# HliasGit/navier_stokes_solver

Measured on AMD Instinct MI355X. Metric: DoF*iters/s (FGMRES+aSIMPLE, Re=100; first K=5 outer iterations), higher is better.
Workload: dtype f64

## Files before the change

### navier_stokes_solver_amd/csrc/nsk_capi.cpp

```cpp
#include <rccl/rccl.h>

#include <algorithm>
#include <cstring>

#include "../../include/nsk_threads.h"
#include <omp.h>
#include "nsk_handle.hpp"
#include "nsk_internal.h"

extern "C" {

int nsk_get_unique_id(void *out128) {
  ncclUniqueId id;
  if (ncclGetUniqueId(&id) != ncclSuccess) return -20;
  std::memcpy(out128, &id, sizeof(id));
  return 0;
}

int nsk_local_group_id(int nranks, void *out128) {
  if (nranks < 1 || !out128) return -1;
  make_local_group(nranks, out128, 0);
  return 0;
}

// ... 45 lines not shown
  S.n = (int)(e - b);
  S.ng = n_ghost;
  S.gbegin = b;
  S.gend = e;
  S.ghost_gid.assign(gids, gids + n_ghost);
  h->support[space].clear();
  h->tF_ok = h->tMp_ok = h->tS_ok = false;
  return 0;
  NSK_CATCH(h)
}

int nsk_set_support_points(nsk_handle h, int space, const double *xy) {
  NSK_TRY(h)
  if (space < 0 || space > 1) throw Error(-50, "nsk_set_support_points: bad space");
  const Space &S = h->sp[space];
  if (xy) h->support[space].assign(xy, xy + 2 * (size_t)S.n);
  else h->support[space].clear();
  h->tF_ok = h->tMp_ok = h->tS_ok = false;
  return 0;
  NSK_CATCH(h)
}

int nsk_set_halo_plan(nsk_handle h, int space, int nn, const int32_t *peer, const int32_t *send_ptr,
                      const int32_t *send_idx, const int32_t *recv_ptr) {
  NSK_TRY_DEV(h)
  if (space < 0 || space > 1 || nn < 0) throw Error(-52, "nsk_set_halo_plan: bad arguments");
  Space &S = h->sp[space];
  S.peers.assign(peer, peer + nn);
  S.send_ptr.assign(send_ptr, send_ptr + nn + 1);
  S.recv_ptr.assign(recv_ptr, recv_ptr + nn + 1);
  S.n_send = nn ? send_ptr[nn] : 0;
  for (int k = 0; k < S.n_send; ++k)
    if (send_idx[k] < 0 || send_idx[k] >= S.n) throw Error(-53, "halo plan: send index outside the owned range");
  if (nn && recv_ptr[nn] != S.ng) throw Error(-54, "halo plan: receive counts do not cover the ghost list");
  S.d_send_idx.upload(send_idx, (size_t)S.n_send, h->s());
  S.d_send_buf.alloc((size_t)std::max(1, S.n_send));
  h->ctx.sync();
  return 0;
  NSK_CATCH(h)
}

int nsk_set_block_csr(nsk_handle h, int b, int n_rows, int n_cols, const int32_t *rowptr, const int32_t *col,
                      const double *val) {
  NSK_TRY_DEV(h)
  if (b < 0 || b > NSK_BLK_BT_GHOST) throw Error(-55, "nsk_set_block_csr: bad block id");
  const int rs = (b == NSK_BLK_F || b == NSK_BLK_BT) ? 0 : 1;
  const int cs = (b == NSK_BLK_F || b == NSK_BLK_B) ? 0 : 1;
  const Space &R = h->sp[rs], &Cc = h->sp[cs];
  const int want_rows = b == NSK_BLK_BT_GHOST ? h->sp[0].ng : R.n;
  if (n_rows != want_rows) throw Error(-56, "nsk_set_block_csr: row count does not match the partition");
  if (n_cols != Cc.n + Cc.ng) throw Error(-57, "nsk_set_block_csr: column count does not match owned+ghost");
  const int64_t nnz = rowptr[n_rows];
  for (int i = 0; i < n_rows; ++i)
    if (rowptr[i + 1] < rowptr[i]) throw Error(-58, "nsk_set_block_csr: rowptr not monotone");
  bool bad_col = false;
#pragma omp parallel for schedule(static) reduction(|| : bad_col)
  for (int64_t k = 0; k < nnz; ++k) bad_col = bad_col || col[k] < 0 || col[k] >= n_cols;
  if (bad_col) throw Error(-59, "nsk_set_block_csr: column id out of range");
  Csr &A = h->blk[b];
  Phase ph("hand-off of one block");
  A.n_rows = n_rows;
  A.n_cols = n_cols;
  A.n_own_cols = Cc.n;
  A.nnz = nnz;
  A.h_rowptr.assign(rowptr, rowptr + n_rows + 1);
  A.h_col.resize((size_t)nnz);
#pragma omp parallel for schedule(static)
  for (int64_t c = 0; c < (nnz + (1 << 20) - 1) >> 20; ++c)
    std::memcpy(A.h_col.data() + (c << 20), col + (c << 20), sizeof(int) * (size_t)std::min<int64_t>(1 << 20, nnz - (c << 20)));
  A.rowptr.upload(rowptr, (size_t)n_rows + 1, h->s());
  A.col.upload(col, (size_t)nnz, h->s());
  A.val.upload(val, (size_t)nnz, h->s());
  if (b == NSK_BLK_MP) ++h->mp_values_version;
  ++A.values_version;
  A.release_f32();
  if (b == NSK_BLK_F) h->asmd.mf_valid = false;
  A.lpr = pick_lpr(nnz, n_rows);
  A.present = true;
  A.build_stream_plan(h->s());
  if (b == NSK_BLK_MP) h->index16_for(A, "M_p");
  if (b == NSK_BLK_F) A.build_blocked(2, 2, h->s());
  if (b == NSK_BLK_BT) A.build_blocked(2, 1, h->s());
  if (b == NSK_BLK_B) A.build_blocked(1, 2, h->s());
  h->ctx.sync();
  if (b == NSK_BLK_F || b == NSK_BLK_BT) { h->jrow_ok = h->jblk_ok = false; h->jrow_nblk = h->jblk_nblk = 0; }
  if (b == NSK_BLK_F) {
    h->tF_ok = false;
    h->amgF.clear();
    if (h->amg_active) h->amg_pending = true;
  }
  if (b == NSK_BLK_MP) h->tMp_ok = false;
  if (b == NSK_BLK_B || b == NSK_BLK_BT || b == NSK_BLK_BT_GHOST) { h->s_symbolic = false; h->tS_ok = false; }
  return 0;
  NSK_CATCH(h)
}

int nsk_update_values(nsk_handle h, int b, const double *val) {
  NSK_TRY_DEV(h)
  if (b < 0 || b > NSK_BLK_BT_GHOST || !h->blk[b].present) throw Error(-60, "nsk_update_values: block not set");
  Csr &A = h->blk[b];
  NSK_HIP(hipMemcpyAsync(A.val.p, val, sizeof(double) * (size_t)A.nnz, hipMemcpyHostToDevice, h->s()));
  if (b == NSK_BLK_MP) ++h->mp_values_version;
  if (b == NSK_BLK_F) h->asmd.mf_valid = false;
  ++A.values_version;
  A.refresh_blocked(h->s());
  h->ctx.sync();
  return 0;
  NSK_CATCH(h)
}

int nsk_set_option(nsk_handle h, int opt, double v) {
  NSK_TRY(h)
  switch (opt) {
    case NSK_OPT_TRI_ORDERING: h->tri_ordering = v != 0.0 ? ORDER_MULTICOLOR : ORDER_NATURAL; break;
    case NSK_OPT_SUBDOMAINS: h->subdomains = std::max(1, (int)v); break;
    case NSK_OPT_FUSE_BLOCK_ROW: h->fuse_block_row = v != 0.0; break;
    case NSK_OPT_STREAM_KERNELS: h->use_stream = v != 0.0; break;
    case NSK_OPT_TRI_SYNC_FREE:
      if (v != 0.0 && v != 1.0 && v != 2.0) throw Error(-61, "NSK_OPT_TRI_SYNC_FREE: 0, 1 or 2");
      h->sync_free_mode = (int)v;
      break;
    case NSK_IOPT_FAULT_INJECT:
      h->fault_inject = (int)v;
      h->ctx.mgs_fault = (h->fault_inject & 4) != 0;
      break;
    case NSK_OPT_TRI_LINE_GROUPS:
      if (v != 0.0 && v != 1.0 && v != 2.0) throw Error(-61, "NSK_OPT_TRI_LINE_GROUPS: 0, 1 or 2");
      h->line_groups = (int)v;
      break;
    case NSK_OPT_MASS_ORDERING:
      if (v != -1.0 && v != 0.0 && v != 1.0) throw Error(-61, "NSK_OPT_MASS_ORDERING: -1, 0 or 1");
      h->mp_ordering = (int)v;
      break;
    case NSK_IOPT_GROUP_U:
    case NSK_IOPT_GROUP_P:
      if (v < 1.0 || v > (double)kTriGroupMax) throw Error(-61, "line-group size: 1 .. 3");
      (opt == NSK_IOPT_GROUP_U ? h->group_u : h->group_p) = (int)v;
      break;
    case NSK_IOPT_FUSED_MGS: h->ctx.fused_mgs = v != 0.0; break;
    case NSK_IOPT_GS_ONE_LAUNCH:
      if (v != 0.0 && v != 1.0 && v != 2.0) throw Error(-61, "one-launch Gram-Schmidt sweeps: 0, 1 or 2");
      h->ctx.gs_one_launch = (int)v;
      break;
    case NSK_IOPT_FGMRES_SKIP_UNUSED:
      if (v != 0.0 && v != 1.0) throw Error(-61, "NSK_IOPT_FGMRES_SKIP_UNUSED: 0 or 1");
      h->skip_unused = v != 0.0;
      break;
    case NSK_IOPT_OVERLAP_HALO: h->overlap_halo = v != 0.0; break;
    case NSK_IOPT_TINY_BYTES: h->tF.tiny_bytes = h->tMp.tiny_bytes = h->tS.tiny_bytes = v; break;
    case NSK_OPT_BSR_VELOCITY: h->use_bsr = v != 0.0; break;
    case NSK_OPT_VELOCITY_AMG: h->velocity_amg = v != 0.0; break;
    case NSK_IOPT_TIMEOP_BETWEEN: h->timeop_between = (int)v; break;
    case NSK_IOPT_INDEX16:
      h->index16 = v != 0.0;
      (void)hipSetDevice(h->ctx.device);
      for (int b : {NSK_BLK_MP, NSK_BLK_S})
        if (h->blk[b].present && h->blk[b].stream_ok) h->index16_for(h->blk[b], b == NSK_BLK_S ? "S" : "M_p");
      h->ctx.sync();
      h->tS_ok = h->tMp_ok = false;
      break;
    case NSK_IOPT_HOST_ANALYSIS:
      h->tF.host_analysis = h->tS.host_analysis = h->tMp.host_analysis = v != 0.0;
      h->tF_ok = h->tS_ok = h->tMp_ok = false;
      break;
    case NSK_OPT_BLAS1_PAIRS:
      if (v != -1.0 && v != 0.0 && v != 1.0) throw Error(-61, "NSK_OPT_BLAS1_PAIRS: -1, 0 or 1");
      h->blas1_pairs = (int)v;
      h->ctx.ws.pairs = v < 0.0 ? (h->variant == 0) : (int)v;
      break;
    case NSK_OPT_SCHUR_SIGN:
      if (v != 1.0 && v != -1.0) throw Error(-61, "NSK_OPT_SCHUR_SIGN: +1 or -1");
      h->schur_sign = (int)v;
      break;
    case NSK_OPT_FACTOR_PRECISION:
      if (v != 64.0 && v != 32.0) throw Error(-61, "NSK_OPT_FACTOR_PRECISION: 64 or 32");
      h->factor_precision = (int)v;
      break;
    case NSK_OPT_INNER_MATRIX_PRECISION:
      if (v != 64.0 && v != 32.0) throw Error(-61, "NSK_OPT_INNER_MATRIX_PRECISION: 64 or 32");
      h->inner_matrix_precision = (int)v;
      break;
    case NSK_OPT_INNER_BASIS_PRECISION:
      if (v != 64.0 && v != 32.0) throw Error(-61, "NSK_OPT_INNER_BASIS_PRECISION: 64 or 32");
      h->inner_basis_precision = (int)v;
      break;
    case NSK_OPT_AMG_PRECISION:
      if (v != 64.0 && v != 32.0) throw Error(-61, "NSK_OPT_AMG_PRECISION: 64 or 32");
      h->amg_precision = (int)v;
      break;
    case NSK_OPT_INNER_MATRIX_FREE_F:
      if (v != 0.0 && v != 1.0) throw Error(-61, "NSK_OPT_INNER_MATRIX_FREE_F: 0 or 1");
      h->matrix_free_f = (int)v;
      break;
    case NSK_IOPT_TRI_X_LAYOUT:
      h->x_layout_mode = v == 0.0 ? 0 : 2;
      h->tF_ok = false;
      break;
    case NSK_OPT_INNER_FUSED_GS:
      if (v != 0.0 && v != 1.0 && v != 2.0) throw Error(-61, "NSK_OPT_INNER_FUSED_GS: 0, 1 or 2");
      h->inner_fused_gs = (int)v;
      break;
    case NSK_OPT_OUTER_FUSED_GS: h->outer_fused_gs = v != 0.0; break;
    case NSK_OPT_CG_SINGLE_REDUCTION: h->cg_fused = v != 0.0; break;
    default: throw Error(-61, "nsk_set_option: unknown option");
  }
  h->push_tri_options();
  return 0;
  NSK_CATCH(h)
}

int nsk_setup_preconditioner(nsk_handle h, int type, int variant, double alpha) {
  NSK_TRY_DEV(h)
  h->setup(type, variant, alpha);
  return 0;
  NSK_CATCH_ABORT(h)
}

int nsk_upload_system(nsk_handle h, const double *ru, const double *rp, const double *xu, const double *xp) {
  NSK_TRY_DEV(h)
  h->ensure_pools();
  const size_t bu = sizeof(double) * (size_t)h->n_u(), bp = sizeof(double) * (size_t)h->n_p();
  NSK_HIP(hipMemcpyAsync(h->rhs_b, ru, bu, hipMemcpyHostToDevice, h->s()));
  NSK_HIP(hipMemcpyAsync(h->rhs_b + h->n_u(), rp, bp, hipMemcpyHostToDevice, h->s()));
  NSK_HIP(hipMemcpyAsync(h->x_b, xu, bu, hipMemcpyHostToDevice, h->s()));
  NSK_HIP(hipMemcpyAsync(h->x_b + h->n_u(), xp, bp, hipMemcpyHostToDevice, h->s()));
  h->ctx.sync();
  return 0;
  NSK_CATCH(h)
}

int nsk_solve_resident(nsk_handle h, int solver, double tol, int max_iter, int *iters, double *final_res) {
  NSK_TRY_DEV(h)
  return h->solve_resident(solver, tol, max_iter, iters, final_res);
  NSK_CATCH_ABORT(h)
}

int nsk_download_solution(nsk_handle h, double *xu, double *xp) {
  NSK_TRY_DEV(h)
  NSK_HIP(hipMemcpyAsync(xu, h->x_b, sizeof(double) * (size_t)h->n_u(), hipMemcpyDeviceToHost, h->s()));
  NSK_HIP(hipMemcpyAsync(xp, h->x_b + h->n_u(), sizeof(double) * (size_t)h->n_p(), hipMemcpyDeviceToHost, h->s()));
  h->ctx.sync();
  return 0;
// ... 509 lines not shown
```

### navier_stokes_solver_amd/csrc/nsk_core.cpp

```cpp
#include "nsk_core.hpp"

#include <rccl/rccl.h>

#include <algorithm>
#include <condition_variable>
#include <cstdlib>
#include <map>
#include <memory>
#include <mutex>

namespace nsk {

#define NSK_NCCL(call)                                                                     \
  do {                                                                                     \
    ncclResult_t r__ = (call);                                                             \
    if (r__ != ncclSuccess)                                                                \
      throw ::nsk::Error(-20, std::string(#call) + ": " + ncclGetErrorString(r__));        \
  } while (0)

struct LocalGroup {
  int n = 0;
  std::mutex m;
  std::condition_variable cv;
  int waiting = 0;
// ... 486 lines not shown
      comm.allreduce_sum(slot(ns), 1, stream);
      scalar_sqrt(stream, slot(ns), slot(ns) + 1);
    }
    if (ns >= 0) ++st.reductions;
    st.blas1_bytes += 4.0 * n * mc + 16.0 * n;
    ++gs_launches;
  }
}
void Ctx::multi_add(int n, double *x, double *const *z, const double *y, int m) {
  const int cap = gs_one_launch == 1 ? kMgsMaxVecs : gs_one_launch == 2 ? 16 : 1;
  for (int i0 = 0; i0 < m; i0 += cap) {
    const int mc = std::min(cap, m - i0);
    VecPackAll Z{};
    CoefPack Y{};
    for (int k = 0; k < mc; ++k) { Z.v[k] = z[i0 + k]; Y.y[k] = y[i0 + k]; }
    if (gs_one_launch && vec_multi_add(stream, n, x, Z, Y, mc)) {
      st.blas1_bytes += 8.0 * n * (mc + 2);
      ++gs_launches;
    } else {
      for (int k = 0; k < mc; ++k, ++gs_launches) vec_axpy(stream, n, sref(y[i0 + k]), z[i0 + k], x);
      st.blas1_bytes += 24.0 * n * mc;
    }
  }
}

bool Ctx::mgs_applicable(int n, int nv) const {
  if (!fused_mgs || comm.active() || nv < 1 || nv > kMgsMaxVecs) return false;
  const int G = std::min(n_cu, kMgsThreads);
  return (long)n <= (long)G * kMgsThreads * 12;
}

void Ctx::warn(const std::string &msg) {
  fprintf(stderr, "[nsk] warning: %s\n", msg.c_str());
  if (warn_text) *warn_text = "warning: " + msg;
}

void Ctx::mgs_timed_out() {
  fused_mgs = false;
  ++mgs_fallbacks;
  if (mgs_err.p) NSK_HIP(hipMemsetAsync(mgs_err.p, 0, sizeof(int), stream));
  warn("one-launch Gram-Schmidt sweep: a wait ran out of spins (workgroups not co-resident: another process on the "
       "GPU?); this column is redone link by link and the sweep stays off for this handle (slower, same results)");
}

bool Ctx::mgs_sweep(int n, double *w, double *const *v, int nv, int so) {
  if (!mgs_applicable(n, nv)) return false;
  const int G = std::min(n_cu, kMgsThreads);
  const size_t tab = (size_t)(kMgsMaxVecs + 1) * G;
  if (mgs_grid != G) {
    mgs_tables.alloc(2 * tab);
    vec_fill_sentinel(stream, (int)(2 * tab), mgs_tables.p);
    mgs_err.alloc(1);
    NSK_HIP(hipMemsetAsync(mgs_err.p, 0, sizeof(int), stream));
    mgs_grid = G;
    mgs_parity = 0;
  }
  MgsArgs A{};
  A.n = n;
  A.nv = nv;
  for (int k = 0; k < nv; ++k) A.v[k] = v[k];
  A.aux = w;
  A.table = mgs_tables.p + (size_t)mgs_parity * tab;
  A.rearm = mgs_tables.p + (size_t)(1 - mgs_parity) * tab;
  A.out = slot(so);
  A.err = mgs_err.p;
  A.fault = mgs_fault ? 1 : 0;
  NSK_HIP(hipMemsetAsync(slot(so + nv + 2), 0, sizeof(double), stream));
  mgs_tier = nsk::mgs_sweep(stream, A, G);
  if (!mgs_tier) return false;
  mgs_parity = 1 - mgs_parity;
  st.reductions += nv + 1;
  st.blas1_bytes += 8.0 * n * (nv + 2);
  return true;
}

int Csr::spmv_launch(hipStream_t s, SpmvForm f, const double *xo, const double *xg, double *y, int mode, const double *z,
                     int c0, int c1) const {
  if (f == SpmvForm::csr_vector) return nsk::spmv(s, view(), lpr, xo, xg, y, mode, z);
  if (c1 == kToPlanEnd) c1 = is_blk(f) ? blk_nblk : nblk;
  if (c1 <= c0) return 0;
  const int *cb = off16.p ? colbase.p + c0 : nullptr;
  switch (f) {
    case SpmvForm::blk_f32:
      nsk::spmv_blk_stream(s, blk_view32(), blk_rowblk.p + c0, c1 - c0, xo, xg, y, mode == 2 ? z : nullptr);
      return 0;
    case SpmvForm::blk: nsk::spmv_blk_stream(s, blk_view(), blk_R, blk_C, blk_rowblk.p + c0, c1 - c0, xo, xg, y); return 0;
    case SpmvForm::stream_f32: {
      const int vec = nsk::spmv_stream(s, view32(), rowblk.p + c0, c1 - c0, even_rows, xo, xg, y, off16.p, cb, mode, z);
      if (vec < 0) throw Error(-1, "fp32 stream SpMV: modes 1 and 2 have no kernel on 16-bit column offsets");
      return vec;
    }
    default: return nsk::spmv_stream(s, view(), rowblk.p + c0, c1 - c0, even_rows, xo, xg, y, mode, z, off16.p, cb);
  }
}

void Ctx::spmv(Csr &A, Space &colspace, const DVec &x, double *y, int mode, const double *z) {
  comm.halo_exchange(colspace, x, stream);
  A.spmv_launch(stream, A.spmv_form(true, false, mode), x.own, x.ghost, y, mode, z);
  ++st.spmv_calls;
  st.spmv_bytes += (double)A.spmv_bytes() + (mode ? 8.0 * A.n_rows : 0.0);
}

bool build_rowblocks(const int *ra, const int *rb, int n_rows, int max_nnz, const std::vector<int> *cuts,
                     std::vector<int> &rowblk, const unsigned char *glue) {
  rowblk.clear();
  rowblk.push_back(0);
  size_t ci = 0;
  int r0 = 0;
  auto nnz_of = [&](int a, int b) { return (ra[b] - ra[a]) + (rb ? rb[b] - rb[a] : 0); };
  while (r0 < n_rows) {
    while (cuts && ci < cuts->size() && (*cuts)[ci] <= r0) ++ci;
    const int limit = (cuts && ci < cuts->size()) ? std::min(n_rows, (*cuts)[ci]) : n_rows;
    int r1 = r0 + 1;
    if (nnz_of(r0, r1) > max_nnz) return false;
    while (r1 < limit && r1 - r0 < kStreamRows && nnz_of(r0, r1 + 1) <= max_nnz) ++r1;
    if (glue) {
      while (r1 < limit && r1 > r0 && glue[r1]) --r1;
      if (r1 == r0) {
        r1 = r0 + 1;
        while (r1 < limit && glue[r1]) ++r1;
        if (r1 - r0 > kStreamRows || nnz_of(r0, r1) > max_nnz) return false;
      }
    }
    rowblk.push_back(r1);
    r0 = r1;
  }
  return true;
}

void Csr::find_interior() {
  int_r0 = int_r1 = 0;
  if (n_cols == n_own_cols) { int_r1 = n_rows; return; }
  std::vector<char> ghost((size_t)n_rows, 0);
#pragma omp parallel for schedule(static)
  for (int i = 0; i < n_rows; ++i) {
    char g = 0;
    for (int k = h_rowptr[i]; k < h_rowptr[i + 1]; ++k) g |= h_col[k] >= n_own_cols;
    ghost[i] = g;
  }
  int best0 = 0, best1 = 0, start = 0;
  for (int i = 0; i <= n_rows; ++i) {
    if (i == n_rows || ghost[i]) {
      if (i - start > best1 - best0) { best0 = start; best1 = i; }
      start = i + 1;
    }
  }
  int_r0 = best0;
  int_r1 = best1;
}

static void interior_runs(const std::vector<int> &rb, int r0, int r1, int &b0, int &b1) {
  b0 = b1 = 0;
  const int nb = (int)rb.size() - 1;
  for (int b = 0; b < nb; ++b)
    if (rb[b] >= r0 && rb[b + 1] <= r1) {
      if (b1 == b0) b0 = b;
      b1 = b + 1;
    }
}

void Csr::build_stream_plan(hipStream_t s) {
  std::vector<int> rb;
  find_interior();
  std::vector<int> cuts;
  if (int_r0 > 0) cuts.push_back(int_r0);
  if (int_r1 < n_rows && int_r1 > int_r0) cuts.push_back(int_r1);
  stream_ok = n_rows > 0 && build_rowblocks(h_rowptr.data(), nullptr, n_rows, kStreamNnz, cuts.empty() ? nullptr : &cuts, rb);
  if (!stream_ok) { nblk = 0; return; }
  nblk = (int)rb.size() - 1;
  interior_runs(rb, int_r0, int_r1, int_b0, int_b1);
  even_rows = true;
  for (int i = 0; i <= n_rows; ++i)
    if (h_rowptr[i] & 1) { even_rows = false; break; }
  rowblk.upload(rb, s);
  off16.release();
  colbase.release();
  idx16_wide = false;
}

void Csr::build_index16(hipStream_t s, bool want) {
  off16.release();
  colbase.release();
  idx16_wide = false;
  if (!want || !stream_ok || nblk <= 0) return;
  if (nnz <= 0) {
    colbase.alloc((size_t)nblk);
    off16.alloc(8);
    NSK_HIP(hipMemsetAsync(colbase.p, 0, sizeof(int) * (size_t)nblk, s));
    NSK_HIP(hipMemsetAsync(off16.p, 0, 8 * sizeof(unsigned short), s));
    return;
  }
  if (!col.p) return;
  DBuf<int> wide;
  wide.alloc(1);
  colbase.alloc((size_t)nblk);
  NSK_HIP(hipMemsetAsync(wide.p, 0, sizeof(int), s));
  nsk::setup_run_col_base(s, nblk, nullptr, rowblk.p, rowptr.p, col.p, colbase.p, wide.p);
  int w = 0;
  NSK_HIP(hipMemcpyAsync(&w, wide.p, sizeof(int), hipMemcpyDeviceToHost, s));
  NSK_HIP(hipStreamSynchronize(s));
  if (w) {
    idx16_wide = true;
    colbase.release();
    return;
  }
  off16.alloc((size_t)nnz + 8);
  NSK_HIP(hipMemsetAsync(off16.p + nnz, 0, 8 * sizeof(unsigned short), s));
  nsk::setup_run_col_offsets(s, nblk, nullptr, rowblk.p, rowptr.p, col.p, colbase.p, off16.p);
}

void Csr::build_blocked(int R, int C, hipStream_t s) {
  blk_ok = false;
  if (n_rows <= 0 || n_rows % R || n_own_cols % C || n_cols % C) return;
  const int nr = n_rows / R;
  std::vector<int> rp(nr + 1, 0);
  bool ok = true;
#pragma omp parallel for schedule(static) reduction(&& : ok)
  for (int r = 0; r < nr; ++r) {
    const int a0 = h_rowptr[R * r], len = h_rowptr[R * r + 1] - a0;
    bool good = len % C == 0;
    for (int q = 1; good && q < R; ++q) good = h_rowptr[R * r + q + 1] - h_rowptr[R * r + q] == len;
    for (int k = 0; good && k < len; k += C) {
      const int c = h_col[a0 + k];
      good = c % C == 0;
      for (int q = 0; good && q < R; ++q)
        for (int t = 0; good && t < C; ++t) good = h_col[h_rowptr[R * r + q] + k + t] == c + t;
    }
    rp[r + 1] = len / C;
    ok = ok && good;
  }
  if (!ok) return;
  for (int r = 0; r < nr; ++r) rp[r + 1] += rp[r];
  blk_count = rp[nr];
  UVec<int> bcol((size_t)blk_count), bsrc((size_t)blk_count * R * C);
  std::vector<int> rb;
#pragma omp parallel for schedule(static)
  for (int r = 0; r < nr; ++r)
    for (int k = 0; k < rp[r + 1] - rp[r]; ++k) {
      const size_t b = (size_t)rp[r] + k;
      bcol[b] = h_col[h_rowptr[R * r] + C * k] / C;
      for (int q = 0; q < R; ++q)
        for (int t = 0; t < C; ++t) bsrc[(b * R + q) * C + t] = h_rowptr[R * r + q] + C * k + t;
    }
  find_interior();
  const int ib0 = (int_r0 + R - 1) / R, ib1 = int_r1 / R;
  std::vector<int> cuts;
  if (ib0 > 0 && ib0 < nr) cuts.push_back(ib0);
  if (ib1 < nr && ib1 > ib0) cuts.push_back(ib1);
  if (!build_rowblocks(rp.data(), nullptr, nr, kBlkMax, cuts.empty() ? nullptr : &cuts, rb)) return;
  interior_runs(rb, ib0, ib1, blk_int_b0, blk_int_b1);
  blk_R = R;
  blk_C = C;
  blk_rows = nr;
  blk_nblk = (int)rb.size() - 1;
  h_blk_rowptr = rp;
  blk_rowptr.upload(rp, s);
  blk_col.upload(bcol, s);
  blk_src.upload(bsrc, s);
  blk_rowblk.upload(rb, s);
  blk_val.alloc((size_t)blk_count * R * C);
  NSK_HIP(hipStreamSynchronize(s));
  blk_ok = true;
  refresh_blocked(s);
}

void Csr::refresh_blocked(hipStream_t s) {
  if (blk_ok) vec_gather(s, (int)(blk_count * blk_R * blk_C), blk_src.p, val.p, blk_val.p);
}

void Csr::refresh_f32(hipStream_t s, bool count_overflow) {
  const bool want_blk = inner32 == 1 || (amg32 & 1), want_val = inner32 == 2 || (amg32 & 2);
  drop_unused_f32();
  if (!want_blk && !want_val) return;
  if (count_overflow) {
    if (!f32_overflow.p) f32_overflow.alloc(1);
    NSK_HIP(hipMemsetAsync(f32_overflow.p, 0, sizeof(unsigned), s));
  }
  unsigned *ovf = count_overflow ? f32_overflow.p : nullptr;
  if (want_blk) {
    const size_t n = (size_t)blk_count * blk_R * blk_C;
    if (blk_val32.n != n) blk_val32.alloc(n);
    vec_gather(s, (int)n, blk_src.p, val.p, blk_val32.p);
    if (ovf && !want_val) vec_to_float(s, (int)nnz, val.p, nullptr, ovf);
  }
  if (want_val) {
    if (val32.n != (size_t)nnz) val32.alloc((size_t)nnz);
    vec_to_float(s, (int)nnz, val.p, val32.p, ovf);
  }
  val32_version = values_version;
}

double *VecPool::get(bool zero) {
  double *p;
  if (!free_list.empty()) {
    p = free_list.back();
// ... 31 lines not shown
```

### navier_stokes_solver_amd/csrc/nsk_core.hpp

```cpp
#pragma once
#include <hip/hip_runtime.h>

#include <cstdint>
#include <cstdio>
#include <cstring>
#include <memory>
#include <stdexcept>
#include <string>
#include <vector>

#include "nsk_kernels.h"

struct ncclComm;

namespace nsk {

struct Error : std::runtime_error {
  int code;
  Error(int c, const std::string &m) : std::runtime_error(m), code(c) {}
};

#define NSK_HIP(call)                                                                              \
  do {                                                                                             \
    hipError_t e__ = (call);                                                                       \
// ... 13 lines not shown
  }
};
template <class T>
using UVec = std::vector<T, DefaultInitAlloc<T>>;

template <class T>
struct DBuf {
  T *p = nullptr;
  size_t n = 0;
  DBuf() = default;
  DBuf(const DBuf &) = delete;
  DBuf &operator=(const DBuf &) = delete;
  DBuf(DBuf &&o) noexcept : p(o.p), n(o.n) { o.p = nullptr; o.n = 0; }
  DBuf &operator=(DBuf &&o) noexcept {
    if (this != &o) { release(); p = o.p; n = o.n; o.p = nullptr; o.n = 0; }
    return *this;
  }
  ~DBuf() { release(); }
  void release() {
    if (p) (void)hipFree(p);
    p = nullptr;
    n = 0;
  }
  void alloc(size_t count) {
    release();
    n = count;
    if (count) NSK_HIP(hipMalloc((void **)&p, count * sizeof(T)));
  }
  void upload(const T *h, size_t count, hipStream_t s) {
    if (count != n) alloc(count);
    if (count) NSK_HIP(hipMemcpyAsync(p, h, count * sizeof(T), hipMemcpyHostToDevice, s));
  }
  template <class A>
  void upload(const std::vector<T, A> &h, hipStream_t s) { upload(h.data(), h.size(), s); }
};

struct LocalXchg {
  DBuf<double> buf[2];
  hipEvent_t ready[2] = {nullptr, nullptr}, done[2] = {nullptr, nullptr};
  long seq = 0;
  std::vector<const LocalXchg *> peer;
  ~LocalXchg() {
    for (int k = 0; k < 2; ++k) {
      if (ready[k]) (void)hipEventDestroy(ready[k]);
      if (done[k]) (void)hipEventDestroy(done[k]);
    }
  }
};

struct Space {
  int n = 0;
  int ng = 0;
  int64_t gbegin = 0, gend = 0;
  std::vector<int> ghost_gid;
  std::vector<int> peers, send_ptr, recv_ptr;
  DBuf<int> d_send_idx;
  DBuf<double> d_send_buf;
  int n_send = 0;
  std::unique_ptr<LocalXchg> lx;
};

struct DVec {
  double *own = nullptr;
  double *ghost = nullptr;
  int n = 0;
};

enum class SpmvForm { csr_vector, stream, stream_f32, blk, blk_f32 };
inline bool is_f32(SpmvForm f) { return f == SpmvForm::stream_f32 || f == SpmvForm::blk_f32; }
inline bool is_blk(SpmvForm f) { return f == SpmvForm::blk || f == SpmvForm::blk_f32; }
constexpr SpmvForm spmv_form(bool blk_ok, bool stream_ok, int inner32, bool use_stream, bool use_bsr, int mode, bool inner) {
  if (inner && mode == 0 && inner32 == 1 && use_stream && use_bsr && blk_ok) return SpmvForm::blk_f32;
  if (inner && mode == 0 && inner32 == 2 && use_stream && stream_ok && !(blk_ok && use_bsr)) return SpmvForm::stream_f32;
  if (blk_ok && use_stream && use_bsr && mode == 0) return SpmvForm::blk;
  if (stream_ok && use_stream) return SpmvForm::stream;
  return SpmvForm::csr_vector;
}
constexpr SpmvForm amg_spmv_form(bool blk_ok, bool stream_ok, bool amg32, bool use_bsr, int mode, bool aligned16) {
  if (!amg32) return spmv_form(blk_ok, stream_ok, 0, true, false, mode, false);
  if (blk_ok && use_bsr && aligned16 && (mode == 0 || mode == 2)) return SpmvForm::blk_f32;
  if (stream_ok) return SpmvForm::stream_f32;
  return SpmvForm::csr_vector;
}

struct Csr {
  int n_rows = 0, n_cols = 0, n_own_cols = 0;
  int64_t nnz = 0;
  std::vector<int> h_rowptr;
  UVec<int> h_col;
  DBuf<int> rowptr, col;
  DBuf<double> val;
  int lpr = 16;
  bool present = false;
  DBuf<int> rowblk;
  int nblk = 0;
  bool stream_ok = false, even_rows = false;
  void build_stream_plan(hipStream_t s);
  DBuf<unsigned short> off16;
  DBuf<int> colbase;
  bool idx16_wide = false;
  void build_index16(hipStream_t s, bool want);
  int int_r0 = 0, int_r1 = 0, int_b0 = 0, int_b1 = 0, blk_int_b0 = 0, blk_int_b1 = 0;
  void find_interior();
  bool blk_ok = false;
  int blk_R = 1, blk_C = 1, blk_rows = 0, blk_nblk = 0;
  int64_t blk_count = 0;
  std::vector<int> h_blk_rowptr;
  DBuf<int> blk_rowptr, blk_col, blk_src, blk_rowblk;
  DBuf<double> blk_val;
  void build_blocked(int R, int C, hipStream_t s);
  void refresh_blocked(hipStream_t s);
  BlkView blk_view() const { return BlkView{blk_rows, n_own_cols / blk_C, blk_rowptr.p, blk_col.p, blk_val.p}; }
  CsrView view() const { return CsrView{n_rows, n_own_cols, rowptr.p, col.p, val.p}; }
  int inner32 = 0, amg32 = 0;
  DBuf<float> blk_val32, val32;
  long values_version = 0, val32_version = -1;
  DBuf<unsigned> f32_overflow;
  void release_f32() { inner32 = amg32 = 0; blk_val32.release(); val32.release(); f32_overflow.release(); val32_version = -1; }
  void refresh_f32(hipStream_t s, bool count_overflow);
  void drop_unused_f32() {
    if (!(inner32 == 1 || (amg32 & 1))) blk_val32.release();
    if (!(inner32 == 2 || (amg32 & 2))) val32.release();
  }
  bool f32_current() const {
    const bool b = inner32 == 1 || (amg32 & 1), v = inner32 == 2 || (amg32 & 2);
    return val32_version == values_version && (!b || blk_val32.p) && (!v || val32.p);
  }
  BlkView32 blk_view32() const { return BlkView32{blk_rows, n_own_cols / blk_C, blk_rowptr.p, blk_col.p, blk_val32.p}; }
  CsrView32 view32() const { return CsrView32{n_rows, n_own_cols, rowptr.p, col.p, val32.p}; }
  static constexpr int kToPlanEnd = -1;
  SpmvForm spmv_form(bool use_stream, bool use_bsr, int mode = 0, bool inner = false) const {
    return nsk::spmv_form(blk_ok, stream_ok, inner32, use_stream, use_bsr, mode, inner);
  }
  int spmv_launch(hipStream_t s, SpmvForm f, const double *x_own, const double *x_ghost, double *y, int mode = 0,
                  const double *z = nullptr, int c0 = 0, int c1 = kToPlanEnd) const;
  double format_bytes(SpmvForm f) const {
    const double vb = is_f32(f) ? 4.0 : 8.0;
    if (is_blk(f)) return (double)blk_count * (4.0 + vb * blk_R * blk_C) + 4.0 * (blk_rows + 1.0) + 8.0 * n_rows + 8.0 * n_cols;
    const bool index16 = off16.p && f != SpmvForm::csr_vector;
    return (double)spmv_bytes() - (8.0 - vb) * (double)nnz - (index16 ? 2.0 * (double)nnz - 4.0 * nblk : 0.0);
  }
  size_t spmv_bytes() const {
    return (size_t)12 * nnz + 4 * ((size_t)n_rows + 1) + 8 * (size_t)n_rows + 8 * (size_t)n_cols;
  }
};

bool build_rowblocks(const int *rowptr_a, const int *rowptr_b, int n_rows, int max_nnz, const std::vector<int> *cuts,
                     std::vector<int> &rowblk, const unsigned char *glue = nullptr);

inline int pick_lpr(int64_t nnz, int n_rows) {
  const double mean = n_rows > 0 ? (double)nnz / n_rows : 0.0;
  if (mean <= 6) return 4;
  if (mean <= 20) return 8;
  if (mean <= 80) return 16;
  if (mean <= 200) return 32;
  return 64;
}

struct LocalGroup;
struct Comm {
  int rank = 0, nranks = 1;
  ncclComm *comm = nullptr;
  LocalGroup *local = nullptr;
  const double *pub_buf = nullptr;
  const std::vector<int> *pub_peers = nullptr, *pub_send_ptr = nullptr;
  double *h_tmp = nullptr;
  bool on_stream = false;
  int device = 0;
  struct Pub {
    const LocalXchg *x[2] = {nullptr, nullptr};
    const std::vector<int> *peers[2] = {nullptr, nullptr}, *send_ptr[2] = {nullptr, nullptr};
    int parity[2] = {0, 0};
  } pub[2];
  long coll_seq = 0, ar_seq = 0;
  DBuf<double> ar_stage[2];
  hipEvent_t ar_ready[2] = {nullptr, nullptr}, ar_done[2] = {nullptr, nullptr};
  void local_exchange_on_stream(Space *const *sps, const DVec *xs, int count, hipStream_t s);
  bool active() const { return nranks > 1 || comm != nullptr; }
  void init(int rank, int nranks, const void *unique_id, int device_id = 0);
  void destroy();
  void abort_group();
  void allreduce_sum(double *d, int count, hipStream_t s);
  void halo_exchange(Space &sp, const DVec &x, hipStream_t s);
  void halo_exchange2(Space &sa, const DVec &xa, Space &sb, const DVec &xb, hipStream_t s);
};

int make_local_group(int nranks, void *out128, int on_stream = 0);
int abort_local_group(const void *unique_id);

struct Stats {
  double setup_ms = 0, solve_ms = 0;
  long outer_iters = 0, inner_u_its = 0, inner_p_its = 0, prec_applies = 0, spmv_calls = 0, tri_applies = 0,
       reductions = 0, host_syncs = 0, ring_applies = 0,
       columns_skipped = 0;
  double spmv_bytes = 0, tri_bytes = 0, blas1_bytes = 0;
};

struct Ctx {
  hipStream_t stream = nullptr;
  hipStream_t stream2 = nullptr;
  hipEvent_t ev_fork = nullptr, ev_join = nullptr;
  void ensure_stream2();
  int device = 0;
  int n_cu = 256;
  Comm comm;
  ReduceWs ws{};
  DBuf<double> ws_partials;
  DBuf<unsigned> ws_ticket;
  static constexpr int kSlots = 4096;
  DBuf<double> d_scal;
  double *h_scal = nullptr;
  int slot_top = 0;
  Stats st;

  void init(int device_id);
  void destroy();
  int alloc_slots(int k) {
    if (slot_top + k > kSlots) throw Error(-11, "out of device scalar slots");
    const int s = slot_top;
    slot_top += k;
    return s;
  }
// ... 89 lines not shown
```

### navier_stokes_solver_amd/csrc/nsk_debug.cpp

```cpp
#include <algorithm>
#include <cstring>

#include "nsk_handle.hpp"
#include "nsk_internal.h"

namespace {
std::vector<int> shifted(const int32_t *p, size_t n, int64_t base) {
  std::vector<int> v(n);
  for (size_t i = 0; i < n; ++i) {
    const int64_t q = (int64_t)p[i] + base;
    if (q < 0 || q > INT32_MAX) throw Error(-62, "position beyond int32");
    v[i] = (int)q;
  }
  return v;
}
DBuf<int> on_device(const int *h, size_t n) {
  DBuf<int> d;
  d.upload(h, n, nullptr);
  return d;
}
DBuf<double> on_device(const double *h, size_t n) {
  DBuf<double> d;
  d.upload(h, n, nullptr);
  return d;
// ... 229 lines not shown
      const long fallbacks = c.mgs_fallbacks;
      arnoldi_column(c, n, d[0], d.data() + 1, m, so, mode, [&] {
        NSK_HIP(hipMemcpyAsync(d[0], vec[0], sizeof(double) * (size_t)n, hipMemcpyHostToDevice, st));
      });
      if (mode == 0) path = c.mgs_fallbacks == fallbacks ? c.mgs_tier : 0;
      break;
    }
    case NSK_DBG_KRY_DOT3: c.dot3(n, d[0], d[1], d[2], so); break;
    case NSK_DBG_KRY_CG_SCALARS:
      set_slots(7);
      cg_fused_scalars(st, c.slot(so), (int)par[7]);
      break;
    case NSK_DBG_KRY_CG_FUSED_UPDATE:
      set_slots(7);
      vec_cg_fused_update(st, n, c.slot(so), d[0], d[1], d[2], d[3], d[4], d[5]);
      break;
    case NSK_DBG_KRY_CHEBY: vec_cheby_step(st, n, par[0], par[1], d[0], d[1], d[2], d[3], (int)par[2]); break;
    case NSK_DBG_KRY_DENSE_MV: dense_mv(st, n, d[0], d[1], d[2]); break;
    case NSK_DBG_KRY_MULTI_DOT_ALL:
      c.multi_dot_all(n, d[0], d.data() + 1, m, so);
      c.allreduce_slots(so, m);
      break;
    case NSK_DBG_KRY_MULTI_AXPY_ALL:
      set_slots(m);
      c.multi_axpy_all(n, d[0], d.data() + 1, m, so, par[m] != 0.0 ? so + m : -1);
      break;
    case NSK_DBG_KRY_MULTI_ADD: c.multi_add(n, d[0], d.data() + 1, par, m); break;
    case NSK_DBG_KRY_MULTI_DOT_ALL_F32: {
      const bool rider = par[0] != 0.0;
      c.multi_dot_all_f32(n, d[0], f.data() + 1, m, rider, so);
      c.allreduce_slots(so, m + (rider ? 1 : 0));
      break;
    }
    case NSK_DBG_KRY_MULTI_AXPY_ALL_F32:
      set_slots(m);
      c.multi_axpy_all_f32(n, d[0], f.data() + 1, m, so, par[m] != 0.0 ? so + m : -1);
      break;
    case NSK_DBG_KRY_GS_COLUMN_F32: {
      const int mode = (int)par[0];
      if (mode < 1 || mode > 2) throw Error(-61, "nsk_debug_krylov: fp32 basis: Gram-Schmidt mode 1 or 2");
      if (!c.f32_basis_applies(mode)) throw Error(-61, "nsk_debug_krylov: fp32 basis: the pair forms only");
      arnoldi_column(c, n, d[0], (double *const *)nullptr, m, so, mode, [] {}, f.data() + 1);
      break;
    }
    case NSK_DBG_KRY_EQU:
      set_slots(1);
      vec_equ(st, n, sref(1.0, nullptr, c.slot(so)), d[0], d[1]);
      break;
    case NSK_DBG_KRY_EQU_F32:
      set_slots(1);
      vec_equ_f32(st, n, sref(1.0, nullptr, c.slot(so)), d[0], f[1], d[2]);
      break;
  }
  int bad_guards = 0;
  for (int k = 0; k < n_vec; ++k) {
    if (is_float(k)) {
      hf.resize((size_t)len[k]);
      bad_guards += fv[k].fetch(hf.data(), c);
      for (int64_t i = 0; i < len[k]; ++i) vec[k][i] = (double)hf[(size_t)i];
    } else {
      bad_guards += dv[k].fetch(vec[k], c);
    }
  }
  memcpy(slots64, c.read_slots(so, 64), sizeof(double) * 64);
  info8[0] = (int32_t)c.red_paths;
  info8[1] = path;
  info8[2] = std::min(c.n_cu, kMgsThreads);
  info8[3] = bad_guards;
  info8[4] = (int32_t)(c.gs_launches - gs_launches);
  for (int k = 5; k < 8; ++k) info8[k] = 0;
  return 0;
  NSK_CATCH(h)
}


int nsk_debug_spmv(nsk_handle h, int form, int lpr, int mode, int misalign, int c0, int c1, const nsk_dbg_spmv_mat *Am,
                   const nsk_dbg_spmv_mat *Bm, double *y, const double *z, const double *d, const double *dinv,
                   int32_t *rowblk_out, int rowblk_cap, int32_t *info) {
  NSK_TRY_DEV(h)
  Ctx &c = h->ctx;
  hipStream_t st = h->s();
  for (int k = 0; k < 16; ++k) info[k] = 0;
  info[0] = -1;
  if (form < NSK_DBG_SPMV_CSRV || form > NSK_DBG_SPMV_BLK22_RES_F32) throw Error(-65, "nsk_debug_spmv: unknown form");
  const bool two = form == NSK_DBG_SPMV_STREAM2 || form == NSK_DBG_SPMV_BLK_FUSED;
  const bool res = form == NSK_DBG_SPMV_BLK22_RES || form == NSK_DBG_SPMV_BLK22_RES_F32;
  const bool modes = form == NSK_DBG_SPMV_CSRV || form == NSK_DBG_SPMV_STREAM || form == NSK_DBG_SPMV_STREAM_I16 ||
                     form == NSK_DBG_SPMV_STREAM_F32 || res;
  const bool epi = form == NSK_DBG_SPMV_BLK21_EPI;
  if (!Am || !y || two != (Bm != nullptr)) throw Error(-61, "nsk_debug_spmv: matrices");
  if (mode < 0 || mode > 2 || (mode != 0 && !modes) || (mode == 2 && !z) || (res && mode != 2)) throw Error(-61, "nsk_debug_spmv: mode");
  if (epi && !(d && dinv)) throw Error(-61, "nsk_debug_spmv: the epilogue needs d and dinv");
  if ((two || form == NSK_DBG_SPMV_CSRV) && c0 >= 0) throw Error(-61, "nsk_debug_spmv: this form runs whole plans only");
  int R = 1, C = 1;
  if (form == NSK_DBG_SPMV_BLK22 || form == NSK_DBG_SPMV_BLK22_F32 || form == NSK_DBG_SPMV_BLK_FUSED || res) R = C = 2;
  if (form == NSK_DBG_SPMV_BLK21 || epi) R = 2;
  if (form == NSK_DBG_SPMV_BLK12) C = 2;
  const bool blocked = form >= NSK_DBG_SPMV_BLK22 && form != NSK_DBG_SPMV_STREAM2 && form != NSK_DBG_SPMV_STREAM_I16 && form != NSK_DBG_SPMV_STREAM_I16_F32;
  if ((misalign & 4) && R == 2) throw Error(-61, "nsk_debug_spmv: the R = 2 forms store pairs, y is 16-byte aligned");
  if (two && Bm->n_rows != Am->n_rows) throw Error(-61, "nsk_debug_spmv: both matrices over the same rows");

  Csr A, B;
  dbg_fill_csr(A, *Am, st);
  if (two) dbg_fill_csr(B, *Bm, st);
  info[2] = A.lpr;
  info[3] = R;
  info[4] = C;
  info[5] = A.stream_ok;
  info[6] = A.stream_ok && A.even_rows;

  std::vector<int> rb;
  const std::vector<int> *ea = &A.h_rowptr, *eb = nullptr;
  DBuf<int> fused_rb;
  const int *d_rb = nullptr;
  int ib0 = 0, ib1 = 0, refused = 0;
  auto download = [&](const DBuf<int> &src, int nblk) {
    rb.resize((size_t)nblk + 1);
    NSK_HIP(hipMemcpyAsync(rb.data(), src.p, sizeof(int) * rb.size(), hipMemcpyDeviceToHost, st));
    c.sync();
    d_rb = src.p;
  };
  const bool i16 = form == NSK_DBG_SPMV_STREAM_I16 || form == NSK_DBG_SPMV_STREAM_I16_F32;
  if (form == NSK_DBG_SPMV_STREAM || form == NSK_DBG_SPMV_STREAM_F32 || i16) {
    if (!A.stream_ok) refused = 1;
    else { download(A.rowblk, A.nblk); ib0 = A.int_b0; ib1 = A.int_b1; }
    if (!refused && i16) {
      A.build_index16(st, true);
      if (!A.off16.p) refused = 5;
    }
  } else if (form == NSK_DBG_SPMV_STREAM2) {
    if (!A.even_rows) refused = 3;
    else if (!fused_row_plan(A, B, rb)) refused = 4;
    else { eb = &B.h_rowptr; fused_rb.upload(rb, st); d_rb = fused_rb.p; ib1 = (int)rb.size() - 1; }
  } else if (blocked) {
    A.build_blocked(R, C, st);
    if (two) B.build_blocked(2, 1, st);
    info[7] = A.blk_ok && (!two || B.blk_ok);
    if (!info[7] || (two && A.blk_rows != B.blk_rows)) refused = 2;
    else if (two) {
      if (!fused_blk_plan(A, B, rb)) refused = 4;
      else { ea = &A.h_blk_rowptr; eb = &B.h_blk_rowptr; fused_rb.upload(rb, st); d_rb = fused_rb.p; ib1 = (int)rb.size() - 1; }
    } else { download(A.blk_rowblk, A.blk_nblk); ea = &A.h_blk_rowptr; ib0 = A.blk_int_b0; ib1 = A.blk_int_b1; }
  }
  info[15] = refused;
  if (refused) return 1;
  const int nblk = (int)rb.size() - 1;
  if (form != NSK_DBG_SPMV_CSRV) {
    info[8] = nblk;
    info[9] = ib0;
    info[10] = ib1;
    for (int b = 0; b < nblk; ++b) {
      const int e = (*ea)[rb[b + 1]] - (*ea)[rb[b]] + (eb ? (*eb)[rb[b + 1]] - (*eb)[rb[b]] : 0);
      info[11] = std::max(info[11], rb[b + 1] - rb[b]);
      info[12] = std::max(info[12], e);
    }
    if (rowblk_out) std::copy(rb.begin(), rb.begin() + std::min<size_t>(rb.size(), (size_t)std::max(0, rowblk_cap)), rowblk_out);
    if (c0 < 0) { c0 = 0; c1 = nblk; }
    if (c0 > c1 || c1 > nblk) throw Error(-61, "nsk_debug_spmv: run range");
  }

  const int og = misalign & 1, ob = (misalign >> 1) & 1, oy = (misalign >> 2) & 1;
  DbgVec<double> xa, xag, xb, xbg, yv, zv, dv, div;
  xa.put(Am->x_own, (size_t)A.n_own_cols, kDbgFront, kDbgBack, st);
  xag.put(Am->x_ghost, (size_t)(A.n_cols - A.n_own_cols), kDbgFront + og, kDbgBack, st);
  if (two) {
    xb.put(Bm->x_own, (size_t)B.n_own_cols, kDbgFront + ob, kDbgBack, st);
    xbg.put(Bm->x_ghost, (size_t)(B.n_cols - B.n_own_cols), kDbgFront + og, kDbgBack, st);
  }
  yv.put(y, (size_t)A.n_rows, kDbgFront + oy, kDbgBack, st);
  if (z) zv.put(z, (size_t)A.n_rows, kDbgFront + oy, kDbgBack, st);
  if (epi) { dv.put(d, (size_t)A.n_rows, kDbgFront, kDbgBack, st); div.put(dinv, (size_t)A.n_rows, kDbgFront, kDbgBack, st); }

  const int n_run = c1 - c0;
  switch (form) {
    case NSK_DBG_SPMV_CSRV:
      if (lpr == 0) lpr = A.lpr;
      if (lpr != 2 && lpr != 4 && lpr != 8 && lpr != 16 && lpr != 32 && lpr != 64) throw Error(-61, "nsk_debug_spmv: lpr");
      info[2] = nsk::spmv(st, A.view(), lpr, xa.p, xag.p, yv.p, mode, zv.p);
      break;
    case NSK_DBG_SPMV_STREAM: case NSK_DBG_SPMV_STREAM_I16:
      info[1] = A.spmv_launch(st, SpmvForm::stream, xa.p, xag.p, yv.p, mode, zv.p, c0, c1);
      break;
    case NSK_DBG_SPMV_STREAM_F32: case NSK_DBG_SPMV_STREAM_I16_F32:
      A.inner32 = 2;
      A.refresh_f32(st, false);
      info[1] = A.spmv_launch(st, SpmvForm::stream_f32, xa.p, xag.p, yv.p, mode, zv.p, c0, c1);
      break;
    case NSK_DBG_SPMV_BLK22: case NSK_DBG_SPMV_BLK21: case NSK_DBG_SPMV_BLK12: case NSK_DBG_SPMV_BLK11:
      A.spmv_launch(st, SpmvForm::blk, xa.p, xag.p, yv.p, 0, nullptr, c0, c1);
      break;
    case NSK_DBG_SPMV_BLK22_F32:
      A.inner32 = 1;
      A.refresh_f32(st, false);
      A.spmv_launch(st, SpmvForm::blk_f32, xa.p, xag.p, yv.p, 0, nullptr, c0, c1);
      break;
    case NSK_DBG_SPMV_BLK22_RES:
      nsk::spmv_blk22_residual(st, A.blk_view(), d_rb + c0, n_run, xa.p, xag.p, yv.p, zv.p);
      break;
    case NSK_DBG_SPMV_BLK22_RES_F32:
      A.amg32 = 1;
      A.refresh_f32(st, false);
      A.spmv_launch(st, SpmvForm::blk_f32, xa.p, xag.p, yv.p, 2, zv.p, c0, c1);
      break;
    case NSK_DBG_SPMV_BLK21_EPI:
      nsk::spmv_blk_stream(st, A.blk_view(), 2, 1, d_rb + c0, n_run, xa.p, xag.p, yv.p, dv.p, div.p);
      break;
    case NSK_DBG_SPMV_STREAM2:
      info[1] = nsk::spmv2_stream(st, A.view(), xa.p, xag.p, B.view(), xb.p, xbg.p, d_rb, nblk, yv.p);
      break;
    case NSK_DBG_SPMV_BLK_FUSED:
      nsk::spmv_blk_fused22_21(st, A.blk_view(), xa.p, xag.p, B.blk_view(), xb.p, xbg.p, d_rb, nblk, yv.p);
      break;
  }
  NSK_HIP(hipGetLastError());
  info[0] = form;
  info[14] = form == NSK_DBG_SPMV_CSRV ? 0 : n_run;
  int bad = yv.fetch(y, c);
  for (DbgVec<double> *v : {&xa, &xag, &xb, &xbg, &zv, &dv, &div}) bad += v->fetch(nullptr, c);
  info[13] = bad;
  return 0;
  NSK_CATCH(h)
}

int nsk_debug_tri(nsk_handle h, const nsk_dbg_tri_args *a, int32_t *info) {
  NSK_TRY_DEV(h)
  Ctx &c = h->ctx;
  hipStream_t st = h->s();
  for (int k = 0; k < 40; ++k) info[k] = 0;
  if (!a || a->n < 1 || !a->rowptr || !a->col || !a->val || a->rowptr[0] != 0 || a->n_apply < 1 || !a->b || !a->x ||
      !a->perm_out || !a->factor_out)
    throw Error(-61, "nsk_debug_tri: arguments");
  if (a->kind < 0 || a->kind > 1 || a->ordering < ORDER_NATURAL || a->ordering > ORDER_MULTICOLOR || a->group < 1)
    throw Error(-61, "nsk_debug_tri: kind, ordering or group");
  const int n = a->n;
  for (int i = 0; i < n; ++i)
    if (a->rowptr[i + 1] < a->rowptr[i]) throw Error(-58, "nsk_debug_tri: rowptr not monotone");
  const int64_t nnz = a->rowptr[n];
  for (int i = 0; i < n; ++i)
    for (int k = a->rowptr[i]; k < a->rowptr[i + 1]; ++k)
      if (a->col[k] < 0 || a->col[k] >= n || (k > a->rowptr[i] && a->col[k - 1] >= a->col[k]))
        throw Error(-59, "nsk_debug_tri: column ids out of range or not sorted");
  std::vector<int> sub;
  if (a->n_sub > 1) {
    if (!a->sub_off || a->sub_off[0] != 0 || a->sub_off[a->n_sub] != n) throw Error(-61, "nsk_debug_tri: sub-domain offsets");
    for (int k = 0; k < a->n_sub; ++k)
      if (a->sub_off[k + 1] < a->sub_off[k]) throw Error(-61, "nsk_debug_tri: sub-domain offsets");
    sub.assign(a->sub_off, a->sub_off + a->n_sub + 1);
  }
  if (a->x_layout != 0 && !(a->want_block2 && a->sync_free)) {
    info[16] = 1;
    return 1;
  }

  Csr A;
  A.n_rows = A.n_cols = A.n_own_cols = n;
  A.nnz = nnz;
  A.h_rowptr.assign(a->rowptr, a->rowptr + n + 1);
  A.h_col.assign(a->col, a->col + nnz);
  A.rowptr.upload(a->rowptr, (size_t)n + 1, st);
  A.col.upload(a->col, (size_t)nnz, st);
  A.val.upload(a->val, (size_t)nnz, st);
  A.present = true;

  TriSolve T;
  T.use_stream = a->use_stream != 0;
  T.sync_free = a->sync_free != 0;
  T.tiny_bytes = a->tiny_bytes;
  T.host_analysis = a->host_analysis != 0;
  T.want_index16 = a->want_index16 != 0;
  T.want_f32 = a->want_f32 != 0;
  T.x_layout = a->x_layout != 0 ? 1 : 0;
  T.analyze(&c, A, a->kind, a->ordering, sub, a->want_block2 != 0, a->xy, a->group);
  T.y.alloc((size_t)n + 1 + kDbgBack);
  NSK_HIP(hipMemsetAsync(T.y.p, 0xFF, sizeof(double) * T.y.n, st));
  if (T.x_layout) {
    T.xc.alloc((size_t)n + 1 + kDbgBack);
    NSK_HIP(hipMemsetAsync(T.xc.p, 0xFF, sizeof(double) * T.xc.n, st));
  }
  T.numeric(A.val.p);
  NSK_HIP(hipGetLastError());

  std::vector<DbgVec<double>> bv((size_t)a->n_apply), xv((size_t)a->n_apply);
  for (int k = 0; k < a->n_apply; ++k) {
    bv[k].put(a->b + (size_t)k * n, (size_t)n, kDbgFront, kDbgBack, st);
    xv[k].put(a->x + (size_t)k * n, (size_t)n, kDbgFront, kDbgBack, st);
  }
  for (int k = 0; k < a->n_apply; ++k) T.apply(bv[k].p, xv[k].p);
  NSK_HIP(hipGetLastError());
  int bad = 0;
  for (int k = 0; k < a->n_apply; ++k) {
    bad += xv[k].fetch(a->x + (size_t)k * n, c);
    bad += bv[k].fetch(nullptr, c);
  }
  for (const DBuf<double> *iv : {&T.y, &T.xc}) {
    if (iv->n != (size_t)n + 1 + kDbgBack) continue;
    std::vector<double> tail(kDbgBack);
    NSK_HIP(hipMemcpyAsync(tail.data(), iv->p + n + 1, sizeof(double) * kDbgBack, hipMemcpyDeviceToHost, st));
    c.sync();
    for (double v : tail) {
      uint64_t bits;
      memcpy(&bits, &v, 8);
      bad += bits != ~0ull;
// ... 149 lines not shown
```

### navier_stokes_solver_amd/csrc/nsk_handle.hpp

```cpp
#pragma once
#include <chrono>
#include <exception>
#include <string>
#include <vector>

#include "../../include/nsk.h"
#include "nsk_solver.hpp"
#include "nsk_amg.hpp"
#include "nsk_assembly.hpp"
#include "nsk_tri.hpp"

using namespace nsk;

inline double wall_ms() {
  return std::chrono::duration<double, std::milli>(std::chrono::steady_clock::now().time_since_epoch()).count();
}
inline bool verbose() {
  static const bool v = getenv("NSK_VERBOSE") && atoi(getenv("NSK_VERBOSE")) > 0;
  return v;
}
struct Phase {
  const char *name;
  double t0;
  explicit Phase(const char *n) : name(n), t0(wall_ms()) {}
// ... 185 lines not shown
    double mf_nu = 0, mf_inv_dt = 0;
    int mf_stokes = 0;
    DBuf<double> d0, mf_wk;
    bool forces_set = false;
    long n_faces = 0;
    DBuf<int> face_cell;
    DBuf<unsigned char> face_side;
    DBuf<double> face_tab, force_slots, force_out;
    bool record_set = false;
    long rec_cells = 0;
    int rec_sub = 1;
    DBuf<int> rec_cell;
    DBuf<double> rec_wu, rec_wp, rec_out;
  } asmd;
  int matrix_free_f = 0;
  bool matfree_wanted = false;
  bool matfree_warned = false;
  const char *matfree_obstacle() const {
    if (asmd.simplex) return "the handle assembles P2/P1 triangles";
    if (ctx.comm.nranks > 1) return "the handle is one of several ranks";
    if (subdomains > 1) return "NSK_OPT_SUBDOMAINS > 1";
    if (!asmd.ready || !asmd.mf_valid) return "block (0,0) does not hold the values of the last nsk_assemble";
    return nullptr;
  }
  bool matfree_in_effect() const { return matfree_wanted && inner_solve_on(NSK_BLK_F) && !matfree_obstacle(); }
  void matfree_check(const char *who) const {
    if (asmd.simplex || ctx.comm.nranks > 1) throw Error(-65, std::string(who) + ": matrix-free F covers congruent Q3/Q2 cells on one rank only");
    if (!asmd.ready || !asmd.mf_valid)
      throw Error(-66, std::string(who) + ": block (0,0) does not hold the values of a device assembly (call nsk_assemble)");
  }
  double matfree_bytes() const { return asm_matfree_F_bytes(asm_view(), asmd.mf_stokes); }
  void matfree_apply(const DVec &x, double *y) {
    {
      Sampled smp(sampler, NSK_BLK_F, s());
      asm_matfree_F(s(), asm_view(), asmd.cq.p, asmd.mf_nu, asmd.mf_inv_dt, asmd.mf_stokes, asmd.d0.p, x.own, x.ghost,
                    asmd.mf_wk.p, y);
    }
    ++ctx.st.spmv_calls;
    ctx.st.spmv_bytes += matfree_bytes();
  }
  AsmMesh asm_view() const {
    return AsmMesh{asmd.n_cells, sp[0].n / 2, sp[1].n, asmd.cell_of_dof0, asmd.cell_u.p, asmd.cell_p.p, asmd.cell_flags.p,
                   asmd.node_cells.p, asmd.node_off.p, asmd.node_self.p, asmd.pdof_cells.p, asmd.dirichlet.p,
                   asmd.tables.p};
  }

  int n_u() const { return sp[0].n; }
  int n_p() const { return sp[1].n; }
  int N() const { return sp[0].n + sp[1].n; }
  DVec ub(double *base) const { return DVec{base, base + N(), n_u()}; }
  DVec pb(double *base) const { return DVec{base + n_u(), base + N() + sp[0].ng, n_p()}; }
  DVec bb(double *base) const { return DVec{base, base + N(), N()}; }
  hipStream_t s() { return ctx.stream; }

  void ensure_pools() {
    if (pools_ready) return;
    if (!blk[NSK_BLK_F].present || !blk[NSK_BLK_B].present) throw Error(-40, "set blocks F and B before this call");
    pool_u.init(&ctx, sp[0].n, sp[0].ng);
    pool_p.init(&ctx, sp[1].n, sp[1].ng);
    pool_b.init(&ctx, N(), sp[0].ng + sp[1].ng);
    rhs_b = pool_b.get(true);
    x_b = pool_b.get(true);
    pools_ready = true;
  }
  void halo(int space, const DVec &x) { ctx.comm.halo_exchange(sp[space], x, s()); }
  bool inner_solve_on(int b) const {
    if (prec_type < 0) return false;
    if (b == NSK_BLK_F) return prec_type != 2 || variant == 0;
    if (b == NSK_BLK_MP) return prec_type != 2;
    if (b == NSK_BLK_S) return prec_type == 2 && variant == 0;
    return false;
  }
  SpmvForm form_of(const Csr &A, int mode = 0, bool inner = false) const { return A.spmv_form(use_stream != 0, use_bsr != 0, mode, inner); }
  int inner_width(const Csr &A) const { return is_f32(form_of(A, 0, true)) ? 4 : 8; }
  void spmv_nohalo(Csr &A, const DVec &x, double *y, int mode = 0, const double *z = nullptr, bool inner = false) {
    {
      Sampled smp(sampler, (int)(&A - blk), s());
      A.spmv_launch(s(), form_of(A, mode, inner), x.own, x.ghost, y, mode, z);
    }
    ++ctx.st.spmv_calls;
    ctx.st.spmv_bytes += (double)A.spmv_bytes() + (mode == 1 ? 8.0 * A.n_rows : 0.0);
  }
  bool index16 = true;
  void index16_for(Csr &A, const char *name) {
    A.build_index16(s(), index16);
    if (verbose() && index16 && A.stream_ok && !A.off16.p)
      fprintf(stderr, "[nsk] %s: a run of the stream plan spans 65 536 columns or more — int32 column ids stay in use\n", name);
  }
  bool overlap_halo = true;
  long overlapped_spmvs = 0;
  void spmv_halo(Csr &A, int space, const DVec &x, double *y) {
    if (matfree_wanted && &A == &blk[NSK_BLK_F]) {
      const char *why = matfree_obstacle();
      if (!why) {
        halo(space, x);
        matfree_apply(x, y);
        return;
      }
      if (!matfree_warned) {
        matfree_warned = true;
        fprintf(stderr, "[nsk] warning: NSK_OPT_INNER_MATRIX_FREE_F = 1, but %s: the inner FGMRES multiplies by the assembled F\n", why);
      }
    }
    const SpmvForm form = form_of(A, 0, true);
    if (is_f32(form) && A.val32_version != A.values_version) A.refresh_f32(s(), false);
    const bool blocked = is_blk(form);
    const int b0 = blocked ? A.blk_int_b0 : A.int_b0, b1 = blocked ? A.blk_int_b1 : A.int_b1;
    const int nb = blocked ? A.blk_nblk : A.nblk;
    EventSampler::Slot *smp = sampler.find((int)(&A - blk));
    const bool sampling = smp && smp->used < smp->cap;
    if (!overlap_halo || ctx.comm.nranks <= 1 || form == SpmvForm::csr_vector || b1 <= b0 || sampling) {
      halo(space, x);
      spmv_nohalo(A, x, y, 0, nullptr, true);
      return;
    }
    if (smp) ++smp->seen;
    ++overlapped_spmvs;
    ctx.ensure_stream2();
    auto part = [&](hipStream_t st, int c0, int c1) { A.spmv_launch(st, form, x.own, x.ghost, y, 0, nullptr, c0, c1); };
    NSK_HIP(hipEventRecord(ctx.ev_fork, s()));
    NSK_HIP(hipStreamWaitEvent(ctx.stream2, ctx.ev_fork, 0));
    part(ctx.stream2, b0, b1);
    NSK_HIP(hipEventRecord(ctx.ev_join, ctx.stream2));
    halo(space, x);
    part(s(), 0, b0);
    part(s(), b1, nb);
    NSK_HIP(hipStreamWaitEvent(s(), ctx.ev_join, 0));
    ++ctx.st.spmv_calls;
    ctx.st.spmv_bytes += (double)A.spmv_bytes();
  }
  void jacobian_vmult(const DVec &xb, double *yb) {
    const DVec xu = ub(xb.own), xp = pb(xb.own);
    ctx.comm.halo_exchange2(sp[0], xu, sp[1], xp, s());
    Csr &F = blk[NSK_BLK_F], &Bt = blk[NSK_BLK_BT], &B = blk[NSK_BLK_B];
    const bool blocked = use_stream && use_bsr && F.blk_ok && Bt.blk_ok && F.blk_R == 2 && Bt.blk_R == 2 &&
                         F.blk_rows == Bt.blk_rows;
    if (fuse_block_row && blocked && !jblk_ok && jblk_nblk == 0) {
      std::vector<int> rb;
      if (fused_blk_plan(F, Bt, rb)) {
        jblk_nblk = (int)rb.size() - 1;
        jblk_blk.upload(rb, s());
        ctx.sync();
        jblk_ok = true;
      } else jblk_nblk = -1;
    }
    if (fuse_block_row && use_stream && !jrow_ok && jrow_nblk == 0 && F.even_rows) {
      std::vector<int> rb;
      if (fused_row_plan(F, Bt, rb)) {
        jrow_nblk = (int)rb.size() - 1;
        jrow_blk.upload(rb, s());
        ctx.sync();
        jrow_ok = true;
      } else jrow_nblk = -1;
    }
    const double fused_bytes = (double)F.spmv_bytes() + (double)Bt.spmv_bytes() - 8.0 * F.n_rows - 4.0 * (F.n_rows + 1);
    if (fuse_block_row && blocked && jblk_ok) {
      nsk::spmv_blk_fused22_21(s(), F.blk_view(), xu.own, xu.ghost, Bt.blk_view(), xp.own, xp.ghost, jblk_blk.p,
                               jblk_nblk, yb);
      ctx.st.spmv_calls += 2;
      ctx.st.spmv_bytes += fused_bytes;
    } else if (fuse_block_row && use_stream && jrow_ok) {
      nsk::spmv2_stream(s(), F.view(), xu.own, xu.ghost, Bt.view(), xp.own, xp.ghost, jrow_blk.p, jrow_nblk, yb);
      ctx.st.spmv_calls += 2;
      ctx.st.spmv_bytes += fused_bytes;
    } else {
      spmv_nohalo(F, xu, yb, 0);
      spmv_nohalo(Bt, xp, yb, 1);
    }
// ... 83 lines not shown
```

### navier_stokes_solver_amd/csrc/nsk_internal.h

```cpp
#pragma once
#include <stdint.h>

enum {
  NSK_IOPT_TRI_X_LAYOUT = 6,
  NSK_IOPT_FAULT_INJECT = 100,
  NSK_IOPT_GROUP_U = 103,
  NSK_IOPT_GROUP_P = 104,
  NSK_IOPT_TINY_BYTES = 102,
  NSK_IOPT_OVERLAP_HALO = 107,
  NSK_IOPT_HOST_ANALYSIS = 108,
  NSK_IOPT_TIMEOP_BETWEEN = 109,
  NSK_IOPT_INDEX16 = 110,
  NSK_IOPT_GS_ONE_LAUNCH = 111,
  NSK_IOPT_FGMRES_SKIP_UNUSED = 112,
  NSK_IOPT_FUSED_MGS = 106
};

#ifdef __cplusplus
extern "C" {
#endif
int nsk_debug_tri_trace(struct nsk_handle_s *h, int which, int64_t *out16, int max_runs, int *grid);
int nsk_local_group_id_mode(int nranks, int on_stream, void *out128);
int nsk_abort_local_group(const void *uid128);
int nsk_debug_tri_ordering(int n, const int32_t *rowptr, const int32_t *col, int n_sub, const int32_t *sub_off,
                           int want_block2, const double *xy, int group, int32_t *perm_out, int32_t *info4,
                           uint8_t *chain_out);
int nsk_debug_ilu0_at_offset(int what, int n, const int32_t *rowptr, const int32_t *col, double *val_inout, int64_t base);
int nsk_debug_schur_at_offset(int n_p, int n_u, const int32_t *b_rp, const int32_t *b_col, const double *b_val,
                              const double *dinv, const int32_t *bt_rp, const int32_t *bt_col, const double *bt_val,
                              const int32_t *s_rp, const int32_t *s_col, double *s_val_out, int64_t base);
enum {
  NSK_DBG_KRY_DOT = 0, NSK_DBG_KRY_NORM2 = 1, NSK_DBG_KRY_AXPY_DOT = 2, NSK_DBG_KRY_AXPY_NORM2 = 3, NSK_DBG_KRY_CG_UPDATE = 4,
  NSK_DBG_KRY_MULTI_DOT = 5, NSK_DBG_KRY_MULTI_AXPY = 6, NSK_DBG_KRY_GS_COLUMN = 7, NSK_DBG_KRY_DOT3 = 8,
  NSK_DBG_KRY_CG_SCALARS = 9, NSK_DBG_KRY_CG_FUSED_UPDATE = 10, NSK_DBG_KRY_CHEBY = 11, NSK_DBG_KRY_DENSE_MV = 12,
  NSK_DBG_KRY_MULTI_DOT_ALL = 13, NSK_DBG_KRY_MULTI_AXPY_ALL = 14, NSK_DBG_KRY_MULTI_ADD = 15,
  NSK_DBG_KRY_MULTI_DOT_ALL_F32 = 16, NSK_DBG_KRY_MULTI_AXPY_ALL_F32 = 17, NSK_DBG_KRY_GS_COLUMN_F32 = 18,
  NSK_DBG_KRY_EQU = 19, NSK_DBG_KRY_EQU_F32 = 20
};
int nsk_debug_krylov(struct nsk_handle_s *h, int op, int n, int m, int offset, const double *par, int n_vec,
                     double *const *vec, const int64_t *len, double *slots64, int32_t *info8);
enum {
  NSK_DBG_SPMV_CSRV = 0, NSK_DBG_SPMV_STREAM = 1, NSK_DBG_SPMV_STREAM_F32 = 2, NSK_DBG_SPMV_BLK22 = 3,
  NSK_DBG_SPMV_BLK21 = 4, NSK_DBG_SPMV_BLK12 = 5, NSK_DBG_SPMV_BLK11 = 6, NSK_DBG_SPMV_BLK22_F32 = 7,
  NSK_DBG_SPMV_BLK21_EPI = 8, NSK_DBG_SPMV_STREAM2 = 9, NSK_DBG_SPMV_BLK_FUSED = 10, NSK_DBG_SPMV_STREAM_I16 = 11,
  NSK_DBG_SPMV_STREAM_I16_F32 = 12, NSK_DBG_SPMV_BLK22_RES = 13, NSK_DBG_SPMV_BLK22_RES_F32 = 14
};
struct nsk_dbg_spmv_mat {
  int32_t n_rows, n_cols, n_own_cols, pad_;
  const int32_t *rowptr, *col;
  const double *val, *x_own, *x_ghost;
};
int nsk_debug_spmv(struct nsk_handle_s *h, int form, int lpr, int mode, int misalign, int c0, int c1,
                   const struct nsk_dbg_spmv_mat *A, const struct nsk_dbg_spmv_mat *B, double *y, const double *z,
                   const double *d, const double *dinv, int32_t *rowblk_out, int rowblk_cap, int32_t *info16);
struct nsk_dbg_tri_args {
  int32_t n, kind, ordering, n_sub;
  const int32_t *rowptr, *col;
  const double *val;
  const int32_t *sub_off;
  const double *xy;
  int32_t group, want_block2, use_stream, sync_free;
  double tiny_bytes;
  int32_t host_analysis, want_index16, want_f32, x_layout;
  int32_t n_apply, pad_;
  const double *b;
  double *x;
  int32_t *perm_out;
  double *factor_out;
};
int nsk_debug_tri(struct nsk_handle_s *h, const struct nsk_dbg_tri_args *a, int32_t *info40);
enum {
  NSK_DBG_AMG_SCAN = 0, NSK_DBG_AMG_BLOCK = 1, NSK_DBG_AMG_DIAG = 2, NSK_DBG_AMG_STRENGTH = 3, NSK_DBG_AMG_MIS_PULL = 4,
  NSK_DBG_AMG_MIS_DECIDE = 5, NSK_DBG_AMG_MIS_MARK = 6, NSK_DBG_AMG_ROOTS = 7, NSK_DBG_AMG_JOIN = 8,
  NSK_DBG_AMG_AGG_WEIGHTS = 9, NSK_DBG_AMG_AGGREGATE = 10, NSK_DBG_AMG_PRODUCT = 11, NSK_DBG_AMG_PRODUCT_COUNT = 12,
  NSK_DBG_AMG_TRANSPOSE = 13, NSK_DBG_AMG_ROWS_SORT = 14, NSK_DBG_AMG_START_VECTOR = 15
};
struct nsk_dbg_amg_mat {
  int32_t n_rows, n_cols;
  const int32_t *rowptr, *col;
  const double *val;
};
struct nsk_dbg_amg_args {
  int32_t op, n, r0, r1, pass, stamp, roots_only, first, product, first_tier, nc, out_cap;
  int64_t flag_words;
  double threshold, c;
  struct nsk_dbg_amg_mat A, B;
  const int32_t *i_in;
  const uint64_t *key, *key2;
  const uint16_t *flag;
  const double *ad, *dinv, *pw;
  int32_t *i_out;
  uint64_t *k_out;
  uint16_t *flag_out;
  double *d_out, *d_out2;
  int32_t *out_rp, *out_col;
  double *out_val;
  int64_t *out64;
};
int nsk_debug_amg(struct nsk_handle_s *h, const struct nsk_dbg_amg_args *a, int32_t *info16);
int nsk_debug_index_width(struct nsk_handle_s *h, int b, int32_t *out3);
int nsk_debug_spmv_form(int blk_ok, int stream_ok, int inner32, int use_stream, int use_bsr, int mode, int inner);
int nsk_debug_amg_spmv_form(int blk_ok, int stream_ok, int amg32, int use_bsr, int mode, int aligned16);
int64_t nsk_debug_amg_level(struct nsk_handle_s *h, int shard, int level, int which, int32_t *rowptr, int32_t *col, double *val,
                            double *dinv_or_inverse);
int nsk_debug_amg_forms(struct nsk_handle_s *h, int64_t *out5);
int nsk_debug_pool_counts(struct nsk_handle_s *h, int32_t *out6);
enum { NSK_DBG_ASM_CQ = 0, NSK_DBG_ASM_D0 = 1, NSK_DBG_ASM_NODE_CELLS = 2, NSK_DBG_ASM_NODE_OFF = 3,
       NSK_DBG_ASM_NODE_SELF = 4, NSK_DBG_ASM_PDOF_CELLS = 5 };
int64_t nsk_debug_asm(struct nsk_handle_s *h, int what, void *out, int64_t cap);
#ifdef __cplusplus
}
#endif
```

### navier_stokes_solver_amd/csrc/nsk_kernels.h

```cpp
#pragma once
#include <hip/hip_runtime.h>
#include <stdint.h>

namespace nsk {

struct SRef {
  double c;
  const double *num;
  const double *den;
};
inline SRef sref(double c) { return SRef{c, nullptr, nullptr}; }
inline SRef sref(double c, const double *num) { return SRef{c, num, nullptr}; }
inline SRef sref(double c, const double *num, const double *den) { return SRef{c, num, den}; }

struct ReduceWs {
  double *partials;
  unsigned *ticket;
  int pairs;
};
constexpr int kMaxReduceBlocks = 512;
constexpr int kMaxReduceOut = 32;

template <class V>
struct CsrViewT {
  int n_rows;
  int n_own_cols;
  const int *rowptr;
  const int *col;
  const V *val;
};
using CsrView = CsrViewT<double>;
using CsrView32 = CsrViewT<float>;
int spmv(hipStream_t s, const CsrView &A, int lanes_per_row, const double *x_own, const double *x_ghost, double *y,
         int mode, const double *z);

constexpr int kStreamNnz = 2048;
constexpr int kStreamRows = 64;
int spmv_stream(hipStream_t s, const CsrView &A, const int *rowblk, int nblk, int even_rows, const double *x_own,
                const double *x_ghost, double *y, int mode, const double *z, const unsigned short *off16 = nullptr,
                const int *colbase = nullptr);
int spmv_stream(hipStream_t s, const CsrView32 &A, const int *rowblk, int nblk, int even_rows, const double *x_own,
                const double *x_ghost, double *y, const unsigned short *off16 = nullptr, const int *colbase = nullptr,
                int mode = 0, const double *z = nullptr);
int spmv2_stream(hipStream_t s, const CsrView &A, const double *xa_own, const double *xa_ghost, const CsrView &B,
                 const double *xb_own, const double *xb_ghost, const int *rowblk, int nblk, double *y);

template <class V>
struct BlkViewT {
  int n_brows;
  int n_own_bcols;
  const int *rowptr;
  const int *col;
  const V *val;
};
using BlkView = BlkViewT<double>;
using BlkView32 = BlkViewT<float>;
constexpr int kBlkMax = 1024;
void spmv_blk_stream(hipStream_t s, const BlkView &A, int R, int C, const int *rowblk, int nblk, const double *x_own,
                     const double *x_ghost, double *y, const double *epi_d = nullptr, const double *epi_dinv = nullptr);
void spmv_blk_stream(hipStream_t s, const BlkView32 &A, const int *rowblk, int nblk, const double *x_own,
                     const double *x_ghost, double *y, const double *z = nullptr);
void spmv_blk22_residual(hipStream_t s, const BlkView &A, const int *rowblk, int nblk, const double *x_own,
                         const double *x_ghost, double *y, const double *z);
void spmv_blk_fused22_21(hipStream_t s, const BlkView &A, const double *xa_own, const double *xa_ghost,
                         const BlkView &B, const double *xb_own, const double *xb_ghost, const int *rowblk, int nblk,
                         double *y);

void vec_set(hipStream_t s, int n, double *y, double v);
void vec_copy(hipStream_t s, int n, const double *x, double *y);
void vec_equ(hipStream_t s, int n, SRef a, const double *x, double *y);
void vec_axpy(hipStream_t s, int n, SRef a, const double *x, double *y);
void vec_sadd(hipStream_t s, int n, SRef sc, SRef a, const double *x, double *y);
void vec_axpy2(hipStream_t s, int n, SRef a, const double *x, SRef b, const double *z, double *y);
void vec_scale(hipStream_t s, int n, SRef a, double *y);
void vec_mul(hipStream_t s, int n, const double *d, double *y);
void vec_submul(hipStream_t s, int n, const double *d, const double *x, double *y);
void vec_sub_then_mul(hipStream_t s, int n, const double *x, const double *d, double *y);
void vec_recip(hipStream_t s, int n, const double *x, double *y);
void vec_cheby_step(hipStream_t s, int n, double c1, double c2, const double *dinv, const double *r, double *w,
                    double *x, int set_x);
void dense_mv(hipStream_t s, int n, const double *M, const double *b, double *x);
constexpr int kRedScalar = 1, kRedPairs = 2;
int vec_dot(hipStream_t s, const ReduceWs &ws, int n, const double *x, const double *y, double *out, int want_sqrt);
int vec_axpy_dot(hipStream_t s, const ReduceWs &ws, int n, SRef a, const double *x, double *y, const double *w,
                 double *out, int want_sqrt);
int vec_cg_update(hipStream_t s, const ReduceWs &ws, int n, SRef a, const double *d, const double *h, double *x,
                  double *g, double *out);
struct VecPack {
  const double *v[8];
};
int vec_multi_dot(hipStream_t s, const ReduceWs &ws, int n, const double *w, const VecPack &P, int m, double *out);
void gs_pythagoras(hipStream_t s, double *h, int m);
int vec_multi_axpy(hipStream_t s, const ReduceWs &ws, int n, double *w, const VecPack &P, int m, const double *h,
                   double *norm_out);
constexpr int kMgsThreads = 1024, kMgsMaxVecs = 32;
struct VecPackAll {
  const double *v[kMgsMaxVecs];
};
int vec_multi_dot_all(hipStream_t s, const ReduceWs &ws, int n, const double *w, const VecPackAll &P, int m, double *out);
int vec_multi_axpy_all(hipStream_t s, const ReduceWs &ws, int n, double *w, const VecPackAll &P, int m, const double *h,
                       double *norm_out);
struct CoefPack {
  double y[kMgsMaxVecs];
};
int vec_multi_add(hipStream_t s, int n, double *x, const VecPackAll &Z, const CoefPack &Y, int m);
struct VecPack32 {
  const float *v[kMgsMaxVecs];
};
int vec_multi_dot_f32(hipStream_t s, const ReduceWs &ws, int n, const double *w, const VecPack32 &P, int m, int rider,
                      double *out);
int vec_multi_axpy_f32(hipStream_t s, const ReduceWs &ws, int n, double *w, const VecPack32 &P, int m, const double *h,
                       double *norm_out);
int red_grid_quads(int n);
void vec_equ_f32(hipStream_t s, int n, SRef a, const double *x, float *v, double *vw);
struct MgsArgs {
  int n, nv;
  const double *v[kMgsMaxVecs];
  double *aux, *table, *rearm, *out;
  int *err;
  int fault;
};
int mgs_sweep(hipStream_t s, const MgsArgs &A, int G);
int vec_dot3(hipStream_t s, const ReduceWs &ws, int n, const double *r, const double *u, const double *w, double *out);
void cg_fused_scalars(hipStream_t s, double *sc7, int first);
void vec_cg_fused_update(hipStream_t s, int n, const double *sc7, const double *u, const double *w, double *p, double *sv,
                         double *x, double *r);
void scalar_sqrt(hipStream_t s, const double *in, double *out);
void vec_gather(hipStream_t s, int n, const int *idx, const double *x, double *y);
void vec_gather(hipStream_t s, int n, const int *idx, const double *x, float *y);
void vec_to_float(hipStream_t s, int n, const double *x, float *y, unsigned *overflow);
void extract_diag(hipStream_t s, const CsrView &A, double *d, double *dinv);

struct TriView {
  int n;
  const int *rowptr;
  const int *diag;
  const int *col;
  const double *val;
  const int *perm;
};
void tri_lower_level(hipStream_t s, const TriView &T, int kind, int lpr, const int *rows, int nrows, const double *rhs,
                     double *y);
void tri_upper_level(hipStream_t s, const TriView &T, int kind, int lpr, const int *rows, int nrows, double *y,
                     double *out);
void tri_lower_serial(hipStream_t s, const TriView &T, int kind, const int *lvl_ptr, const int *rows, int l0, int l1,
                      const double *rhs, double *y);
// ... 19 lines not shown
struct TriBlkT {
  const int *rowptr;
  const int *col;
  const V *val;
  const int4 *desc;
};
using TriBlk = TriBlkT<double>;
using TriBlk32 = TriBlkT<float>;
void tri_blk_level(hipStream_t s, const TriBlk &M, int b0, int b1, int lower, int kind, const double *intra,
                   const int *permn, const double *rhs, double *x);
void tri_blk_level(hipStream_t s, const TriBlk32 &M, int b0, int b1, int lower, int kind, const double *intra,
                   const int *permn, const double *rhs, double *x);
void invert_node_diagonals(hipStream_t s, int n_nodes, double *intra);

void vec_fill_sentinel(hipStream_t s, int n, double *y);
constexpr int kTriGroupMax = 3;
template <class V>
struct TriChainT {
  int gmax;
  const unsigned char *chain;
  const V *cpl;
};
using TriChain = TriChainT<double>;
using TriChain32 = TriChainT<float>;
void tri_stream_syncfree(hipStream_t s, const TriHalf &M, int n_blocks, int lower, int kind, int run_nnz,
                         int wrong_order , const double *dinv, const int *perm, const double *rhs,
                         const double *own, double *w, double *reset ,
                         int *err, long long *dbg = nullptr ,
                         TriChain chain = TriChain{1, nullptr, nullptr});
void tri_stream_syncfree(hipStream_t s, const TriHalf32 &M, int n_blocks, int lower, int kind, int run_nnz,
                         int wrong_order, const double *dinv, const int *perm, const double *rhs, const double *own,
                         double *w, double *reset, int *err, long long *dbg, TriChain32 chain);
void tri_blk_syncfree(hipStream_t s, const TriBlk &M, int n_blocks, int lower, int kind, int permx,
                      int wrong_order , const double *intra, const int *permn, const double *rhs,
                      const double *own, double *w, double *out, double *reset, int *err,
                      TriChain chain = TriChain{1, nullptr, nullptr});
void tri_blk_syncfree(hipStream_t s, const TriBlk32 &M, int n_blocks, int lower, int kind, int permx, int wrong_order,
                      const double *intra, const int *permn, const double *rhs, const double *own, double *w,
                      double *out, double *reset, int *err, TriChain32 chain);
void vec_gather_or_zero(hipStream_t s, long n, const int *idx, const double *x, double *y);
void vec_gather_or_zero(hipStream_t s, long n, const int *idx, const double *x, float *y);


constexpr int kRingGroups = 2, kRingWaves = 8, kRingThreads = 64 * kRingWaves * kRingGroups, kRingLpr = 2, kRingRegs = 8;
constexpr int kRingRowsPerWave = 64 / kRingLpr, kRingRows = kRingWaves * kRingRowsPerWave;
constexpr int kRingSlots = 16384;
constexpr int kRingDepth = 2;
constexpr int kRingStep = 12;
constexpr int kRingMaxEpoch = 48;
constexpr int kRingMaxRows = 1 << 26;
struct RingHalf {
  int n_pass;
  int epoch;
  const uint4 *hdr;
  const char *ent;
  const char *rowrec;
  const int2 *rearm;
};
void tri_ring(hipStream_t s, const RingHalf &R, int lower, int kind, const double *own, double *dst);
void ring_fill_values(hipStream_t s, long n, const int *idx, const double *x, char *dst, int stride);
struct TouchRanges { const char *p[6]; size_t bytes[6]; };
void mem_touch(hipStream_t s, const TouchRanges &R, unsigned *sink);

void ilu0_factor_level(hipStream_t s, int n_level_rows, const int *rows, const int *rowptr, const int *diag,
                       const int *col, double *val, int max_row_nnz);
void ilu0_factor_serial(hipStream_t s, const int *lvl_ptr, const int *rows, int l0, int l1, const int *rowptr,
                        const int *diag, const int *col, double *val, int max_row_nnz);

void spgemm_bdbt_numeric(hipStream_t s, const CsrView &B, const double *dinv_own, const double *dinv_ghost,
                         const CsrView &Bt, const CsrView &Btg, const int *s_rowptr, const int *s_col, double *s_val,
                         int n_rows, int max_row_nnz);

void setup_permute_rows(hipStream_t s, int n, const int *a_rowptr, const int *a_col, const int *perm, const int *iperm,
                        const int *prp, int *pcol, int *psrc, int *pdiag, int max_row, int *err);
void setup_blk_count(hipStream_t s, int nn, const int *prp, const int *pcol, int max_blocks, int *cnt_l, int *cnt_u);
void setup_blk_fill(hipStream_t s, int nn, const int *prp, const int *pcol, const int *perm, int x_layout, int max_blocks,
                    const int *lrp, const int *urp, int *lcol, int *lsrc, int *ucol, int *usrc, int *isrc, int *permn);
void setup_csr_fill(hipStream_t s, int n, const int *prp, const int *pcol, const int *pdiag, const int *perm, int max_row,
                    const int *lrp, const int *urp, int *lcol, int *lsrc, int *ucol, int *usrc);
void setup_run_col_base(hipStream_t s, int nb, const int4 *desc, const int *rowblk, const int *rowptr, const int *col,
                        int *base, int *wide);
void setup_run_col_offsets(hipStream_t s, int nb, const int4 *desc, const int *rowblk, const int *rowptr, const int *col,
                           const int *base, unsigned short *off);

void halo_pack(hipStream_t s, int n, const int *idx, const double *x, double *buf);
constexpr int kLocalSumMax = 16;
struct LocalSumArgs {
  int n;
  const double *src[kLocalSumMax];
};
void local_sum(hipStream_t s, int count, const LocalSumArgs &A, double *out);

}
```

### navier_stokes_solver_amd/csrc/nsk_kernels.hip

```cpp
#include "nsk_kernels.h"

#include <algorithm>
#include <type_traits>

namespace nsk {

namespace {

constexpr int BLK = 256;

__device__ __forceinline__ double sval(const SRef &s) {
  double v = s.c;
  if (s.num) v *= *s.num;
  if (s.den) v /= *s.den;
  return v;
}

template <int W>
__device__ __forceinline__ double subwave_sum(double v) {
#pragma unroll
  for (int off = W / 2; off > 0; off >>= 1) v += __shfl_down(v, off, W);
  return v;
}

inline int ew_grid(int n) {
  long b = ((long)n + BLK * 4 - 1) / (BLK * 4);
  if (b < 1) b = 1;
  if (b > 2048) b = 2048;
  return (int)b;
}
constexpr int RBLK = 1024;
inline int red_grid(int n) {
  long b = ((long)n + RBLK * 4 - 1) / (RBLK * 4);
  if (b < 1) b = 1;
  if (b > kMaxReduceBlocks) b = kMaxReduceBlocks;
  return (int)b;
}
inline int red_grid_pairs(int n, int cap) {
  long b = (((long)n + 1) / 2 + RBLK * 4 - 1) / (RBLK * 4);
  if (b < 1) b = 1;
  if (b > cap) b = cap;
  return (int)b;
}

template <int LPR, int MODE>
__global__ __launch_bounds__(BLK) void spmv_kernel(CsrView A, const double *__restrict__ xo,
                                                   const double *__restrict__ xg, double *__restrict__ y,
                                                   const double *__restrict__ z) {
  const long tid = (long)blockIdx.x * BLK + threadIdx.x;
  const int row = (int)(tid / LPR);
  const int lane = (int)(tid % LPR);
  double s = 0.0;
  if (row < A.n_rows) {
    const int re = A.rowptr[row + 1];
    for (int k = A.rowptr[row] + lane; k < re; k += LPR) {
      const int c = A.col[k];
      const double xv = c < A.n_own_cols ? xo[c] : xg[c - A.n_own_cols];
      s += A.val[k] * xv;
    }
  }
  s = subwave_sum<LPR>(s);
  if (lane == 0 && row < A.n_rows) {
    if (MODE == 0) y[row] = s;
    else if (MODE == 1) y[row] = (z ? z[row] : y[row]) + s;
    else y[row] = z[row] - s;
  }
}

constexpr int RG = 4;

__device__ __forceinline__ double2 widen2(double2 v) { return v; }
__device__ __forceinline__ double2 widen2(float2 v) { return make_double2((double)v.x, (double)v.y); }

template <class I>
struct IdxPair;
template <>
struct IdxPair<int> {
  typedef int v2 __attribute__((ext_vector_type(2)));
  typedef v2 unaligned __attribute__((aligned(4)));
  typedef v2 aligned2;
  int a, b;
  __device__ __forceinline__ IdxPair(v2 q, int) : a(q[0]), b(q[1]) {}
};
template <>
struct IdxPair<unsigned short> {
  typedef unsigned v2;
  typedef unsigned unaligned __attribute__((aligned(2)));
  typedef unsigned aligned2;
  int a, b;
  __device__ __forceinline__ IdxPair(unsigned q, int base) : a(base + (int)(q & 0xffffu)), b(base + (int)(q >> 16)) {}
};

template <class V, int VEC, class I = int>
__device__ __forceinline__ void stream_products(const I *__restrict__ col, const V *__restrict__ val, int k0,
                                                int k1, int n_own, const double *__restrict__ xo,
                                                const double *__restrict__ xg, double *prod, int base = 0) {
  if (VEC == 3) {
    constexpr int U = kStreamNnz / (2 * BLK);
    typedef V vv2 __attribute__((ext_vector_type(2)));
    typedef vv2 vd2u __attribute__((aligned(sizeof(V))));
    int c0[U], c1[U];
    double v0[U], v1[U], x0[U], x1[U];
#pragma unroll
    for (int u = 0; u < U; ++u) {
      const int k = k0 + 2 * ((int)threadIdx.x + u * BLK);
      if (k + 1 < k1) {
        const IdxPair<I> ci(*reinterpret_cast<const typename IdxPair<I>::unaligned *>(col + k), base);
        const vv2 vi = *reinterpret_cast<const vd2u *>(val + k);
        c0[u] = ci.a; c1[u] = ci.b; v0[u] = (double)vi[0]; v1[u] = (double)vi[1];
      } else {
        const bool ok = k < k1;
        c0[u] = ok ? base + (int)col[k] : 0; v0[u] = ok ? (double)val[k] : 0.0; c1[u] = 0; v1[u] = 0.0;
      }
    }
#pragma unroll
    for (int u = 0; u < U; ++u) {
      x0[u] = *(c0[u] < n_own ? xo + c0[u] : xg + (c0[u] - n_own));
      x1[u] = *(c1[u] < n_own ? xo + c1[u] : xg + (c1[u] - n_own));
    }
#pragma unroll
    for (int u = 0; u < U; ++u) {
      const int k = k0 + 2 * ((int)threadIdx.x + u * BLK);
      if (k < k1) prod[k - k0] = v0[u] * x0[u];
      if (k + 1 < k1) prod[k - k0 + 1] = v1[u] * x1[u];
    }
  } else if (VEC == 2) {
    constexpr int U = kStreamNnz / (2 * BLK);
    typedef typename std::conditional<std::is_same<V, double>::value, double2, float2>::type V2;
    int2 c[U];
    double2 v[U];
#pragma unroll
    for (int u = 0; u < U; ++u) {
      const int k = k0 + 2 * ((int)threadIdx.x + u * BLK);
      const bool ok = k < k1;
      if (ok) {
        const IdxPair<I> ci(*reinterpret_cast<const typename IdxPair<I>::aligned2 *>(col + k), base);
        c[u] = make_int2(ci.a, ci.b);
      } else c[u] = make_int2(0, 0);
      v[u] = ok ? widen2(*reinterpret_cast<const V2 *>(val + k)) : make_double2(0.0, 0.0);
    }
    double x0[U], x1[U];
#pragma unroll
    for (int u = 0; u < U; ++u) {
      x0[u] = *(c[u].x < n_own ? xo + c[u].x : xg + (c[u].x - n_own));
      x1[u] = *(c[u].y < n_own ? xo + c[u].y : xg + (c[u].y - n_own));
    }
#pragma unroll
    for (int u = 0; u < U; ++u) {
      const int k = k0 + 2 * ((int)threadIdx.x + u * BLK);
      if (k < k1) { prod[k - k0] = v[u].x * x0[u]; prod[k - k0 + 1] = v[u].y * x1[u]; }
    }
  } else {
    constexpr int U = kStreamNnz / BLK;
    int c[U];
    double v[U], xv[U];
#pragma unroll
    for (int u = 0; u < U; ++u) {
      const int k = k0 + (int)threadIdx.x + u * BLK;
      const bool ok = k < k1;
      c[u] = ok ? base + (int)col[k] : 0;
      v[u] = ok ? (double)val[k] : 0.0;
    }
#pragma unroll
    for (int u = 0; u < U; ++u) xv[u] = *(c[u] < n_own ? xo + c[u] : xg + (c[u] - n_own));
#pragma unroll
    for (int u = 0; u < U; ++u) {
      const int k = k0 + (int)threadIdx.x + u * BLK;
      if (k < k1) prod[k - k0] = v[u] * xv[u];
    }
  }
}

__device__ __forceinline__ double row_sum_lds(const double *prod, int b, int e, int lane) {
  double s = 0.0;
  int j = b + lane;
  for (; j + 3 * RG < e; j += 4 * RG) {
    const double a0 = prod[j], a1 = prod[j + RG], a2 = prod[j + 2 * RG], a3 = prod[j + 3 * RG];
    s += a0;
    s += a1;
    s += a2;
    s += a3;
  }
  for (; j < e; j += RG) s += prod[j];
  return subwave_sum<RG>(s);
}

template <class V, int VEC, int MODE, class I = int>
__global__ __launch_bounds__(BLK) void spmv_stream_kernel(CsrViewT<V> A, const int *__restrict__ rowblk,
                                                          const double *__restrict__ xo,
                                                          const double *__restrict__ xg, double *__restrict__ y,
                                                          const double *__restrict__ z,
                                                          const unsigned short *__restrict__ off16 = nullptr,
                                                          const int *__restrict__ colbase = nullptr) {
  __shared__ double prod[kStreamNnz];
  const int r0 = rowblk[blockIdx.x], r1 = rowblk[blockIdx.x + 1];
  constexpr bool I16 = std::is_same<I, unsigned short>::value;
  const int base = I16 ? colbase[blockIdx.x] : 0;
  const int k0 = A.rowptr[r0], k1 = A.rowptr[r1];
  const int r = r0 + (int)threadIdx.x / RG, lane = threadIdx.x % RG;
  const bool have = r < r1;
  int jb = 0, je = 0;
  double zv = 0.0;
  if (have) {
    jb = A.rowptr[r] - k0;
    je = A.rowptr[r + 1] - k0;
    if (MODE == 1) zv = z ? z[r] : y[r];
    if (MODE == 2) zv = z[r];
  }
  if constexpr (I16) stream_products<V, VEC, unsigned short>(off16, A.val, k0, k1, A.n_own_cols, xo, xg, prod, base);
  else stream_products<V, VEC>(A.col, A.val, k0, k1, A.n_own_cols, xo, xg, prod);
  __syncthreads();
  const double sum = row_sum_lds(prod, jb, je, lane);
  if (have && lane == 0) {
    if (MODE == 0) y[r] = sum;
    else if (MODE == 1) y[r] = zv + sum;
    else y[r] = zv - sum;
  }
}

template <int VECA>
__global__ __launch_bounds__(BLK) void spmv2_stream_kernel(CsrView A, const double *__restrict__ xao,
                                                           const double *__restrict__ xag, CsrView B,
                                                           const double *__restrict__ xbo,
                                                           const double *__restrict__ xbg,
                                                           const int *__restrict__ rowblk, double *__restrict__ y) {
  __shared__ double prod[kStreamNnz];
  const int r0 = rowblk[blockIdx.x], r1 = rowblk[blockIdx.x + 1];
  const int a0 = A.rowptr[r0], a1 = A.rowptr[r1], b0 = B.rowptr[r0], b1 = B.rowptr[r1];
  const int r = r0 + (int)threadIdx.x / RG, lane = threadIdx.x % RG;
  const bool have = r < r1;
  int ab = 0, ae = 0, bb = 0, be = 0;
  if (have) {
    ab = A.rowptr[r] - a0; ae = A.rowptr[r + 1] - a0;
    bb = B.rowptr[r] - b0; be = B.rowptr[r + 1] - b0;
  }
  stream_products<double, VECA>(A.col, A.val, a0, a1, A.n_own_cols, xao, xag, prod);
  double *prodB = prod + (a1 - a0);
  stream_products<double, 1>(B.col, B.val, b0, b1, B.n_own_cols, xbo, xbg, prodB);
  __syncthreads();
  double sum = 0.0;
  for (int j = ab + lane; j < ae; j += RG) sum += prod[j];
  for (int j = bb + lane; j < be; j += RG) sum += prodB[j];
  sum = subwave_sum<RG>(sum);
  if (have && lane == 0) y[r] = sum;
}

template <class V, int R, int C>
__device__ __forceinline__ void blk_products(const BlkViewT<V> &A, int k0, int k1, const double *__restrict__ xo,
                                             const double *__restrict__ xg, double *p0, double *p1) {
  constexpr int U = kBlkMax / BLK;
  if (k0 >= k1) return;
  int m[U];
  double2 a0[U], a1[U];
  double x0[U], x1[U];
#pragma unroll
  for (int u = 0; u < U; ++u) {
    const int k = k0 + (int)threadIdx.x + u * BLK;
    const bool ok = k < k1;
    m[u] = ok ? __builtin_nontemporal_load(A.col + k) : 0;
    const V *v = A.val + (size_t)(R * C) * (ok ? k : k0);
    if constexpr (std::is_same<V, float>::value) {
      static_assert(R == 2 && C == 2, "fp32 values: 2 x 2 blocks only");
      const float4 q = *reinterpret_cast<const float4 *>(v);
      a0[u] = make_double2((double)q.x, (double)q.y); a1[u] = make_double2((double)q.z, (double)q.w);
    } else {
      if (R * C == 4) { a0[u] = *reinterpret_cast<const double2 *>(v); a1[u] = *reinterpret_cast<const double2 *>(v + 2); }
      else if (R * C == 2) { a0[u] = *reinterpret_cast<const double2 *>(v); a1[u] = make_double2(0.0, 0.0); }
      else { a0[u] = make_double2(v[0], 0.0); a1[u] = make_double2(0.0, 0.0); }
    }
  }
#pragma unroll
  for (int u = 0; u < U; ++u) {
    x1[u] = 0.0;
    if (C == 2) {
      if (m[u] < A.n_own_bcols) {
        const double2 xv = *reinterpret_cast<const double2 *>(xo + 2 * (size_t)m[u]);
        x0[u] = xv.x; x1[u] = xv.y;
      } else {
        const size_t g = 2 * (size_t)(m[u] - A.n_own_bcols);
        x0[u] = xg[g]; x1[u] = xg[g + 1];
      }
    } else {
      x0[u] = *(m[u] < A.n_own_bcols ? xo + m[u] : xg + (m[u] - A.n_own_bcols));
    }
  }
#pragma unroll
  for (int u = 0; u < U; ++u) {
    const int k = k0 + (int)threadIdx.x + u * BLK;
    if (k < k1) {
      if (R == 2 && C == 2) { p0[k - k0] = a0[u].x * x0[u] + a0[u].y * x1[u]; p1[k - k0] = a1[u].x * x0[u] + a1[u].y * x1[u]; }
      else if (R == 2 && C == 1) { p0[k - k0] = a0[u].x * x0[u]; p1[k - k0] = a0[u].y * x0[u]; }
      else if (R == 1 && C == 2) p0[k - k0] = a0[u].x * x0[u] + a0[u].y * x1[u];
      else p0[k - k0] = a0[u].x * x0[u];
    }
  }
}

template <class V, int R, int C, int EPI>
__global__ __launch_bounds__(BLK) void spmv_blk_kernel(BlkViewT<V> A, const int *__restrict__ rowblk,
                                                       const double *__restrict__ xo, const double *__restrict__ xg,
                                                       double *__restrict__ y, const double *__restrict__ d,
                                                       const double *__restrict__ dinv) {
  __shared__ double p0[kBlkMax];
  __shared__ double p1[R == 2 ? kBlkMax : 1];
  const int r0 = rowblk[blockIdx.x], r1 = rowblk[blockIdx.x + 1];
  const int k0 = A.rowptr[r0], k1 = A.rowptr[r1];
  const int r = r0 + (int)threadIdx.x / RG, lane = threadIdx.x % RG;
  const bool have = r < r1;
  int jb = 0, je = 0;
  if (have) { jb = A.rowptr[r] - k0; je = A.rowptr[r + 1] - k0; }
  blk_products<V, R, C>(A, k0, k1, xo, xg, p0, p1);
  __syncthreads();
  double s0 = 0.0, s1 = 0.0;
  for (int j = jb + lane; j < je; j += RG) { s0 += p0[j]; if (R == 2) s1 += p1[j]; }
  s0 = subwave_sum<RG>(s0);
  if (R == 2) s1 = subwave_sum<RG>(s1);
  if (have && lane == 0) {
    if (EPI == 1 && R == 2) {
      const double2 yo = *reinterpret_cast<const double2 *>(y + 2 * (size_t)r);
      const double2 dd = *reinterpret_cast<const double2 *>(d + 2 * (size_t)r);
      const double2 di = *reinterpret_cast<const double2 *>(dinv + 2 * (size_t)r);
      s0 = __dmul_rn(__dsub_rn(__dmul_rn(yo.x, dd.x), s0), di.x);
      s1 = __dmul_rn(__dsub_rn(__dmul_rn(yo.y, dd.y), s1), di.y);
    }
    if (EPI == 2 && R == 2) {
      const double2 zz = *reinterpret_cast<const double2 *>(d + 2 * (size_t)r);
      s0 = __dsub_rn(zz.x, s0);
      s1 = __dsub_rn(zz.y, s1);
    }
    if (R == 2) *reinterpret_cast<double2 *>(y + 2 * (size_t)r) = make_double2(s0, s1);
    else y[r] = s0;
  }
}

__global__ __launch_bounds__(BLK) void spmv_blk_fused_kernel(BlkView A, const double *__restrict__ xao,
                                                             const double *__restrict__ xag, BlkView B,
                                                             const double *__restrict__ xbo,
                                                             const double *__restrict__ xbg,
                                                             const int *__restrict__ rowblk, double *__restrict__ y) {
  __shared__ double p0[kBlkMax];
  __shared__ double p1[kBlkMax];
  const int r0 = rowblk[blockIdx.x], r1 = rowblk[blockIdx.x + 1];
  const int a0 = A.rowptr[r0], a1 = A.rowptr[r1], b0 = B.rowptr[r0], b1 = B.rowptr[r1];
  const int r = r0 + (int)threadIdx.x / RG, lane = threadIdx.x % RG;
  const bool have = r < r1;
  int ab = 0, ae = 0, bb = 0, be = 0;
  if (have) {
    ab = A.rowptr[r] - a0; ae = A.rowptr[r + 1] - a0;
    bb = B.rowptr[r] - b0 + (a1 - a0); be = B.rowptr[r + 1] - b0 + (a1 - a0);
  }
  blk_products<double, 2, 2>(A, a0, a1, xao, xag, p0, p1);
  blk_products<double, 2, 1>(B, b0, b1, xbo, xbg, p0 + (a1 - a0), p1 + (a1 - a0));
  __syncthreads();
  double s0 = 0.0, s1 = 0.0;
  for (int j = ab + lane; j < ae; j += RG) { s0 += p0[j]; s1 += p1[j]; }
  for (int j = bb + lane; j < be; j += RG) { s0 += p0[j]; s1 += p1[j]; }
  s0 = subwave_sum<RG>(s0);
  s1 = subwave_sum<RG>(s1);
  if (have && lane == 0) *reinterpret_cast<double2 *>(y + 2 * (size_t)r) = make_double2(s0, s1);
}

template <class V, int LOWER, int KIND, int NNZ, int I16 = 0>
__global__ __launch_bounds__(BLK) void tri_stream_kernel(TriHalfT<V> M, int b0, int nb, const double *__restrict__ dinv,
                                                         const int *__restrict__ perm,
                                                         const double *__restrict__ rhs, double *__restrict__ w) {
  __shared__ double prod[NNZ];
  const int per = (int)gridDim.x >> 3;
  const int mapped = (int)(blockIdx.x & 7) * per + (int)(blockIdx.x >> 3);
  if (mapped >= nb) return;
  const int4 d = M.desc[b0 + mapped];
  const int r0 = d.x, r1 = d.y, k0 = d.z, k1 = d.w;
  const int base = I16 ? M.base[b0 + mapped] : 0;
  const int r = r0 + (int)threadIdx.x / RG, lane = threadIdx.x % RG;
  const bool have = r < r1;
  int jb = 0, je = 0, i = 0;
  double own = 0.0, dv = 1.0;
  if (have) {
    jb = M.rowptr[r] - k0;
    je = M.rowptr[r + 1] - k0;
    i = perm[r];
    own = LOWER ? rhs[i] : w[i];
    if (KIND == 1 || !LOWER) dv = dinv[r];
  }
  {
    constexpr int U = NNZ / BLK;
    int c[U];
    double v[U], g[U];
#pragma unroll
    for (int u = 0; u < U; ++u) {
      const int k = k0 + (int)threadIdx.x + u * BLK;
      const bool ok = k < k1;
      if (I16) c[u] = ok ? base + (int)__builtin_nontemporal_load(M.off16 + k) : 0;
      else c[u] = ok ? __builtin_nontemporal_load(M.col + k) : 0;
      v[u] = ok ? (double)__builtin_nontemporal_load(M.val + k) : 0.0;
// ... 1039 lines not shown
__global__ __launch_bounds__(BLK) void spgemm_kernel(CsrView B, const double *__restrict__ dio,
                                                     const double *__restrict__ dig, CsrView Bt, CsrView Btg,
                                                     const int *__restrict__ srp, const int *__restrict__ scol,
                                                     double *__restrict__ sval, int n_rows, int max_nnz) {
  extern __shared__ double lds[];
  const int wave = threadIdx.x >> 6, lane = threadIdx.x & 63;
  const int i = blockIdx.x * (BLK / 64) + wave;
  if (i >= n_rows) return;
  double *acc = lds + (size_t)wave * max_nnz;
  const int ss = srp[i], se = srp[i + 1];
  for (int k = lane; k < se - ss; k += 64) acc[k] = 0.0;
  __builtin_amdgcn_fence(__ATOMIC_SEQ_CST, "wavefront");
  __builtin_amdgcn_wave_barrier();
  for (int k = B.rowptr[i]; k < B.rowptr[i + 1]; ++k) {
    const int m = B.col[k];
    const bool own = m < B.n_own_cols;
    const double a = B.val[k] * (own ? dio[m] : dig[m - B.n_own_cols]);
    const CsrView &R = own ? Bt : Btg;
    const int mr = own ? m : m - B.n_own_cols;
    const int qe = R.rowptr[mr + 1];
    for (int q = R.rowptr[mr] + lane; q < qe; q += 64) {
      const int j = R.col[q];
      int lo = ss, hi = se;
      while (lo < hi) {
        const int mid = lo + ((hi - lo) >> 1);
        if (scol[mid] < j) lo = mid + 1; else hi = mid;
      }
      acc[lo - ss] += a * R.val[q];
    }
    __builtin_amdgcn_fence(__ATOMIC_SEQ_CST, "wavefront");
    __builtin_amdgcn_wave_barrier();
  }
  for (int k = lane; k < se - ss; k += 64) sval[ss + k] = acc[k];
}

template <int LPR, int MODE>
void launch_spmv(hipStream_t s, const CsrView &A, const double *xo, const double *xg, double *y, const double *z) {
  const long threads = (long)A.n_rows * LPR;
  const int grid = (int)((threads + BLK - 1) / BLK);
  if (grid > 0) hipLaunchKernelGGL((spmv_kernel<LPR, MODE>), dim3(grid), dim3(BLK), 0, s, A, xo, xg, y, z);
}
template <int LPR>
void launch_spmv_mode(hipStream_t s, const CsrView &A, const double *xo, const double *xg, double *y, int mode,
                      const double *z) {
  if (mode == 0) launch_spmv<LPR, 0>(s, A, xo, xg, y, z);
  else if (mode == 1) launch_spmv<LPR, 1>(s, A, xo, xg, y, z);
  else launch_spmv<LPR, 2>(s, A, xo, xg, y, z);
}

template <int KIND, bool LOWER>
void launch_tri_level(hipStream_t s, const TriView &T, int lpr, const int *rows, int nrows, const double *rhs,
                      double *y, double *out) {
  if (nrows <= 0) return;
#define NSK_TRI_CASE(L)                                                                                      \
  case L: {                                                                                                  \
    const int grid = (int)(((long)nrows * L + BLK - 1) / BLK);                                               \
    hipLaunchKernelGGL((tri_level_kernel<L, KIND, LOWER>), dim3(grid), dim3(BLK), 0, s, T, rows, nrows, rhs, y, out); \
  } break;
  switch (lpr) {
    NSK_TRI_CASE(4)
    NSK_TRI_CASE(8)
    NSK_TRI_CASE(16)
    NSK_TRI_CASE(32)
    default: NSK_TRI_CASE(64)
  }
#undef NSK_TRI_CASE
}

}

int spmv(hipStream_t s, const CsrView &A, int lpr, const double *xo, const double *xg, double *y, int mode,
         const double *z) {
  switch (lpr) {
    case 2: launch_spmv_mode<2>(s, A, xo, xg, y, mode, z); return 2;
    case 4: launch_spmv_mode<4>(s, A, xo, xg, y, mode, z); return 4;
    case 8: launch_spmv_mode<8>(s, A, xo, xg, y, mode, z); return 8;
    case 16: launch_spmv_mode<16>(s, A, xo, xg, y, mode, z); return 16;
    case 32: launch_spmv_mode<32>(s, A, xo, xg, y, mode, z); return 32;
    default: launch_spmv_mode<64>(s, A, xo, xg, y, mode, z); return 64;
  }
}

int spmv_stream(hipStream_t s, const CsrView &A, const int *rowblk, int nblk, int even_rows, const double *xo,
                const double *xg, double *y, int mode, const double *z, const unsigned short *off16, const int *colbase) {
  if (nblk <= 0) return 0;
#define NSK_SS(V, M)                                                                                                                   \
  do {                                                                                                                                 \
    if (off16) hipLaunchKernelGGL((spmv_stream_kernel<double, V, M, unsigned short>), dim3(nblk), dim3(BLK), 0, s, A, rowblk, xo, xg, y, z, off16, colbase); \
    else hipLaunchKernelGGL((spmv_stream_kernel<double, V, M, int>), dim3(nblk), dim3(BLK), 0, s, A, rowblk, xo, xg, y, z, off16, colbase); \
  } while (0)
  if (even_rows) {
    if (mode == 0) NSK_SS(2, 0); else if (mode == 1) NSK_SS(2, 1); else NSK_SS(2, 2);
    return 2;
  }
  if (mode == 0) NSK_SS(3, 0); else if (mode == 1) NSK_SS(3, 1); else NSK_SS(3, 2);
  return 3;
#undef NSK_SS
}

int spmv_stream(hipStream_t s, const CsrView32 &A, const int *rowblk, int nblk, int even_rows, const double *xo,
                const double *xg, double *y, const unsigned short *off16, const int *colbase, int mode, const double *z) {
  if (nblk <= 0) return 0;
#define NSK_SS(V, M)                                                                                                                   \
  do {                                                                                                                                 \
    if (off16) hipLaunchKernelGGL((spmv_stream_kernel<float, V, M, unsigned short>), dim3(nblk), dim3(BLK), 0, s, A, rowblk, xo, xg, y, z, off16, colbase); \
    else hipLaunchKernelGGL((spmv_stream_kernel<float, V, M, int>), dim3(nblk), dim3(BLK), 0, s, A, rowblk, xo, xg, y, z, off16, colbase); \
  } while (0)
#define NSK_SM(V, M) hipLaunchKernelGGL((spmv_stream_kernel<float, V, M, int>), dim3(nblk), dim3(BLK), 0, s, A, rowblk, xo, xg, y, z, nullptr, nullptr)
  if (mode != 0 && off16) return -1;
  if (even_rows) {
    if (mode == 0) NSK_SS(2, 0); else if (mode == 1) NSK_SM(2, 1); else NSK_SM(2, 2);
    return 2;
  }
  if (mode == 0) NSK_SS(3, 0); else if (mode == 1) NSK_SM(3, 1); else NSK_SM(3, 2);
  return 3;
#undef NSK_SM
#undef NSK_SS
}

int spmv2_stream(hipStream_t s, const CsrView &A, const double *xao, const double *xag, const CsrView &B,
                 const double *xbo, const double *xbg, const int *rowblk, int nblk, double *y) {
  if (nblk <= 0) return 0;
  hipLaunchKernelGGL((spmv2_stream_kernel<2>), dim3(nblk), dim3(BLK), 0, s, A, xao, xag, B, xbo, xbg, rowblk, y);
  return 2;
}

template <class V>
static void tri_blk_level_t(hipStream_t s, const TriBlkT<V> &M, int b0, int b1, int lower, int kind, const double *intra,
                            const int *permn, const double *rhs, double *x) {
  const int nb = b1 - b0;
  if (nb <= 0) return;
  const int grid = ((nb + 7) / 8) * 8;
#define NSK_TB(L, K) hipLaunchKernelGGL((tri_blk_kernel<V, L, K>), dim3(grid), dim3(BLK), 0, s, M, b0, nb, intra, permn, rhs, x)
  if (lower) { if (kind == 0) NSK_TB(1, 0); else NSK_TB(1, 1); }
  else { if (kind == 0) NSK_TB(0, 0); else NSK_TB(0, 1); }
#undef NSK_TB
}
void tri_blk_level(hipStream_t s, const TriBlk &M, int b0, int b1, int lower, int kind, const double *intra,
                   const int *permn, const double *rhs, double *x) {
  tri_blk_level_t(s, M, b0, b1, lower, kind, intra, permn, rhs, x);
}
void tri_blk_level(hipStream_t s, const TriBlk32 &M, int b0, int b1, int lower, int kind, const double *intra,
                   const int *permn, const double *rhs, double *x) {
  tri_blk_level_t(s, M, b0, b1, lower, kind, intra, permn, rhs, x);
}

void spmv_blk_stream(hipStream_t s, const BlkView &A, int R, int C, const int *rowblk, int nblk, const double *xo,
                     const double *xg, double *y, const double *epi_d, const double *epi_dinv) {
  if (nblk <= 0) return;
  if (epi_d) {
    hipLaunchKernelGGL((spmv_blk_kernel<double, 2, 1, 1>), dim3(nblk), dim3(BLK), 0, s, A, rowblk, xo, xg, y, epi_d, epi_dinv);
    return;
  }
#define NSK_BK(RR, CC) hipLaunchKernelGGL((spmv_blk_kernel<double, RR, CC, 0>), dim3(nblk), dim3(BLK), 0, s, A, rowblk, xo, xg, y, nullptr, nullptr)
  if (R == 2 && C == 2) NSK_BK(2, 2);
  else if (R == 2 && C == 1) NSK_BK(2, 1);
  else if (R == 1 && C == 2) NSK_BK(1, 2);
  else NSK_BK(1, 1);
#undef NSK_BK
}

void spmv_blk_stream(hipStream_t s, const BlkView32 &A, const int *rowblk, int nblk, const double *xo, const double *xg,
                     double *y, const double *z) {
  if (nblk <= 0) return;
  if (z) hipLaunchKernelGGL((spmv_blk_kernel<float, 2, 2, 2>), dim3(nblk), dim3(BLK), 0, s, A, rowblk, xo, xg, y, z, nullptr);
  else hipLaunchKernelGGL((spmv_blk_kernel<float, 2, 2, 0>), dim3(nblk), dim3(BLK), 0, s, A, rowblk, xo, xg, y, nullptr, nullptr);
}

void spmv_blk22_residual(hipStream_t s, const BlkView &A, const int *rowblk, int nblk, const double *xo, const double *xg,
                         double *y, const double *z) {
  if (nblk > 0)
    hipLaunchKernelGGL((spmv_blk_kernel<double, 2, 2, 2>), dim3(nblk), dim3(BLK), 0, s, A, rowblk, xo, xg, y, z, nullptr);
}

void spmv_blk_fused22_21(hipStream_t s, const BlkView &A, const double *xao, const double *xag, const BlkView &B,
                         const double *xbo, const double *xbg, const int *rowblk, int nblk, double *y) {
  if (nblk > 0)
    hipLaunchKernelGGL(spmv_blk_fused_kernel, dim3(nblk), dim3(BLK), 0, s, A, xao, xag, B, xbo, xbg, rowblk, y);
}

template <class V>
static void tri_stream_level_t(hipStream_t s, const TriHalfT<V> &M, int b0, int b1, int lower, int kind, int run_nnz,
                               const double *dinv, const int *perm, const double *rhs, double *w) {
  const int nb = b1 - b0;
  if (nb <= 0) return;
  const int grid = ((nb + 7) / 8) * 8;
#define NSK_TS(L, K, N) hipLaunchKernelGGL((tri_stream_kernel<V, L, K, N>), dim3(grid), dim3(BLK), 0, s, M, b0, nb, dinv, perm, rhs, w)
#define NSK_TSN(L, K)                                            \
  do {                                                           \
    if (M.off16) hipLaunchKernelGGL((tri_stream_kernel<V, L, K, 2048, 1>), dim3(grid), dim3(BLK), 0, s, M, b0, nb, dinv, perm, rhs, w); \
    else if (run_nnz <= 512) NSK_TS(L, K, 512);                  \
    else if (run_nnz <= 1024) NSK_TS(L, K, 1024);                \
    else NSK_TS(L, K, 2048);                                     \
  } while (0)
  if (lower) { if (kind == 0) NSK_TSN(1, 0); else NSK_TSN(1, 1); }
  else { if (kind == 0) NSK_TSN(0, 0); else NSK_TSN(0, 1); }
#undef NSK_TSN
#undef NSK_TS
}
void tri_stream_level(hipStream_t s, const TriHalf &M, int b0, int b1, int lower, int kind, int run_nnz,
                      const double *dinv, const int *perm, const double *rhs, double *w) {
  tri_stream_level_t(s, M, b0, b1, lower, kind, run_nnz, dinv, perm, rhs, w);
}
void tri_stream_level(hipStream_t s, const TriHalf32 &M, int b0, int b1, int lower, int kind, int run_nnz,
                      const double *dinv, const int *perm, const double *rhs, double *w) {
  tri_stream_level_t(s, M, b0, b1, lower, kind, run_nnz, dinv, perm, rhs, w);
}

#define NSK_EW(n, ...)                                                                       \
  do {                                                                                       \
    if ((n) > 0) {                                                                           \
      auto f__ = __VA_ARGS__;                                                                \
      hipLaunchKernelGGL((ew_kernel<decltype(f__)>), dim3(ew_grid(n)), dim3(BLK), 0, s, n, f__); \
    }                                                                                        \
  } while (0)

void vec_set(hipStream_t s, int n, double *y, double v) { NSK_EW(n, [=] __device__(int i) { y[i] = v; }); }
void vec_copy(hipStream_t s, int n, const double *x, double *y) { NSK_EW(n, [=] __device__(int i) { y[i] = x[i]; }); }
void vec_equ(hipStream_t s, int n, SRef a, const double *x, double *y) {
  NSK_EW(n, [=] __device__(int i) { y[i] = sval(a) * x[i]; });
}
void vec_axpy(hipStream_t s, int n, SRef a, const double *x, double *y) {
  NSK_EW(n, [=] __device__(int i) { y[i] += sval(a) * x[i]; });
}
void vec_sadd(hipStream_t s, int n, SRef sc, SRef a, const double *x, double *y) {
  NSK_EW(n, [=] __device__(int i) { y[i] = sval(sc) * y[i] + sval(a) * x[i]; });
}
void vec_axpy2(hipStream_t s, int n, SRef a, const double *x, SRef b, const double *z, double *y) {
  NSK_EW(n, [=] __device__(int i) { y[i] += sval(a) * x[i] + sval(b) * z[i]; });
}
void vec_scale(hipStream_t s, int n, SRef a, double *y) { NSK_EW(n, [=] __device__(int i) { y[i] *= sval(a); }); }
void vec_mul(hipStream_t s, int n, const double *d, double *y) { NSK_EW(n, [=] __device__(int i) { y[i] *= d[i]; }); }
void vec_submul(hipStream_t s, int n, const double *d, const double *x, double *y) {
  NSK_EW(n, [=] __device__(int i) { y[i] -= d[i] * x[i]; });
}
void vec_sub_then_mul(hipStream_t s, int n, const double *x, const double *d, double *y) {
  NSK_EW(n, [=] __device__(int i) { y[i] = (y[i] - x[i]) * d[i]; });
}
void vec_recip(hipStream_t s, int n, const double *x, double *y) {
  NSK_EW(n, [=] __device__(int i) { y[i] = 1.0 / x[i]; });
}
void vec_cheby_step(hipStream_t s, int n, double c1, double c2, const double *dinv, const double *r, double *w,
                    double *x, int set_x) {
  NSK_EW(n, [=] __device__(int i) {
    const double wi = (c1 != 0.0 ? c1 * w[i] : 0.0) + c2 * dinv[i] * r[i];
    w[i] = wi;
    x[i] = set_x ? wi : x[i] + wi;
  });
}

__global__ __launch_bounds__(BLK) void dense_mv_kernel(int n, const double *__restrict__ M, const double *__restrict__ b,
                                                       double *__restrict__ x) {
  const int row = (int)(blockIdx.x * (BLK / 64) + threadIdx.x / 64), lane = threadIdx.x % 64;
  double sum = 0.0;
  if (row < n)
// ... 599 lines not shown
```

### navier_stokes_solver_amd/csrc/nsk_setup_kernels.hip

```cpp
#include "nsk_kernels.h"

namespace nsk {
namespace {
constexpr int SBLK = 256;

__device__ __forceinline__ void wave_lds_sync() {
  __builtin_amdgcn_fence(__ATOMIC_SEQ_CST, "wavefront");
  __builtin_amdgcn_wave_barrier();
}

__global__ __launch_bounds__(SBLK) void permute_rows_kernel(int n, const int *__restrict__ a_rowptr, const int *__restrict__ a_col,
                                                            const int *__restrict__ perm, const int *__restrict__ iperm,
                                                            const int *__restrict__ prp, int *__restrict__ pcol,
                                                            int *__restrict__ psrc, int *__restrict__ pdiag, int max_row,
                                                            int *err) {
  extern __shared__ int lds[];
  const int wave = threadIdx.x >> 6, lane = threadIdx.x & 63;
  const int i = blockIdx.x * (SBLK / 64) + wave;
  if (i >= n) return;
  int *keys = lds + (size_t)wave * max_row;
  const int r = perm[i], b = a_rowptr[r], len = a_rowptr[r + 1] - b, base = prp[i];
  for (int k = lane; k < len; k += 64) keys[k] = iperm[a_col[b + k]];
  wave_lds_sync();
  bool found = false;
// ... 37 lines not shown
    return;
  }
  wave_lds_sync();
  if (lane == 0) permn[r] = perm[2 * r] / 2;
  for (int j = lane; j < nb; j += 64) {
    const int k = 2 * j, me = cid[j], cl = cls[j];
    if (cl == 2) {
      isrc[4 * (size_t)r + 0] = a1 + k;
      isrc[4 * (size_t)r + 1] = a0 + k + 1;
      isrc[4 * (size_t)r + 2] = a0 + k;
      isrc[4 * (size_t)r + 3] = a1 + k + 1;
      continue;
    }
    int rank = 0;
    for (int q = 0; q < nb; ++q) rank += (cls[q] == cl) & (cid[q] < me);
    const size_t w = (size_t)(cl == 0 ? lrp[r] : urp[r]) + rank;
    int *colv = cl == 0 ? lcol : ucol, *srcv = cl == 0 ? lsrc : usrc;
    colv[w] = me;
    srcv[4 * w + 0] = a0 + k;
    srcv[4 * w + 1] = a0 + k + 1;
    srcv[4 * w + 2] = a1 + k;
    srcv[4 * w + 3] = a1 + k + 1;
  }
}

__global__ __launch_bounds__(SBLK) void csr_split_kernel(int n, const int *__restrict__ prp, const int *__restrict__ pcol,
                                                         const int *__restrict__ pdiag, const int *__restrict__ perm,
                                                         int max_row, const int *__restrict__ lrp, const int *__restrict__ urp,
                                                         int *__restrict__ lcol, int *__restrict__ lsrc, int *__restrict__ ucol,
                                                         int *__restrict__ usrc) {
  extern __shared__ int lds[];
  const int wave = threadIdx.x >> 6, lane = threadIdx.x & 63;
  const int i = blockIdx.x * (SBLK / 64) + wave;
  if (i >= n) return;
  int *keys = lds + (size_t)wave * max_row;
  const int b = prp[i], e = prp[i + 1], d = pdiag[i], len = e - b;
  for (int k = lane; k < len; k += 64) keys[k] = perm[pcol[b + k]];
  wave_lds_sync();
  const int dl = d - b;
  for (int k = lane; k < len; k += 64) {
    if (k == dl) continue;
    const int key = keys[k];
    const bool low = k < dl;
    const int q0 = low ? 0 : dl + 1, q1 = low ? dl : len;
    int rank = 0;
    for (int q = q0; q < q1; ++q) rank += keys[q] < key;
    const size_t w = (size_t)(low ? lrp[i] : urp[i]) + rank;
    (low ? lcol : ucol)[w] = key;
    (low ? lsrc : usrc)[w] = b + k;
  }
}

template <int FILL>
__global__ __launch_bounds__(SBLK) void run_index16_kernel(int nb, const int4 *__restrict__ desc, const int *__restrict__ rowblk,
                                                           const int *__restrict__ rowptr, const int *__restrict__ col,
                                                           int *base, unsigned short *__restrict__ off, int *wide) {
  __shared__ int lo[SBLK / 64], hi[SBLK / 64];
  const int b = (int)blockIdx.x;
  if (b >= nb) return;
  const int k0 = desc ? desc[b].z : rowptr[rowblk[b]], k1 = desc ? desc[b].w : rowptr[rowblk[b + 1]];
  if (FILL) {
    const int bs = base[b];
    for (int k = k0 + (int)threadIdx.x; k < k1; k += SBLK) off[k] = (unsigned short)(col[k] - bs);
    return;
  }
  int mn = INT32_MAX, mx = INT32_MIN;
  for (int k = k0 + (int)threadIdx.x; k < k1; k += SBLK) {
    const int c = col[k];
    mn = min(mn, c);
    mx = max(mx, c);
  }
  for (int o = 32; o > 0; o >>= 1) {
    mn = min(mn, __shfl_down(mn, o, 64));
    mx = max(mx, __shfl_down(mx, o, 64));
  }
  if (threadIdx.x % 64 == 0) { lo[threadIdx.x / 64] = mn; hi[threadIdx.x / 64] = mx; }
  __syncthreads();
  if (threadIdx.x == 0) {
    for (int w = 1; w < SBLK / 64; ++w) { mn = min(mn, lo[w]); mx = max(mx, hi[w]); }
    base[b] = k0 < k1 ? mn : 0;
    if (k0 < k1 && (long long)mx - (long long)mn > 65535) *wide = 1;
  }
}
}

void setup_run_col_base(hipStream_t s, int nb, const int4 *desc, const int *rowblk, const int *rowptr, const int *col,
                        int *base, int *wide) {
  if (nb <= 0) return;
  hipLaunchKernelGGL((run_index16_kernel<0>), dim3(nb), dim3(SBLK), 0, s, nb, desc, rowblk, rowptr, col, base, nullptr, wide);
}
void setup_run_col_offsets(hipStream_t s, int nb, const int4 *desc, const int *rowblk, const int *rowptr, const int *col,
                           const int *base, unsigned short *off) {
  if (nb <= 0) return;
  hipLaunchKernelGGL((run_index16_kernel<1>), dim3(nb), dim3(SBLK), 0, s, nb, desc, rowblk, rowptr, col, const_cast<int *>(base), off, nullptr);
}

void setup_permute_rows(hipStream_t s, int n, const int *a_rowptr, const int *a_col, const int *perm, const int *iperm,
                        const int *prp, int *pcol, int *psrc, int *pdiag, int max_row, int *err) {
  if (n <= 0) return;
  const int grid = (n + SBLK / 64 - 1) / (SBLK / 64);
  hipLaunchKernelGGL(permute_rows_kernel, dim3(grid), dim3(SBLK), sizeof(int) * (size_t)max_row * (SBLK / 64), s, n, a_rowptr, a_col, perm,
                     iperm, prp, pcol, psrc, pdiag, max_row, err);
}
void setup_blk_count(hipStream_t s, int nn, const int *prp, const int *pcol, int max_blocks, int *cnt_l, int *cnt_u) {
  if (nn <= 0) return;
  const int grid = (nn + SBLK / 64 - 1) / (SBLK / 64);
  hipLaunchKernelGGL((blk_split_kernel<false>), dim3(grid), dim3(SBLK), sizeof(int) * 2 * (size_t)max_blocks * (SBLK / 64), s, nn, prp, pcol,
                     nullptr, 1, max_blocks, cnt_l, cnt_u, nullptr, nullptr, nullptr, nullptr, nullptr, nullptr, nullptr, nullptr);
}
void setup_blk_fill(hipStream_t s, int nn, const int *prp, const int *pcol, const int *perm, int x_layout, int max_blocks,
                    const int *lrp, const int *urp, int *lcol, int *lsrc, int *ucol, int *usrc, int *isrc, int *permn) {
  if (nn <= 0) return;
  const int grid = (nn + SBLK / 64 - 1) / (SBLK / 64);
  hipLaunchKernelGGL((blk_split_kernel<true>), dim3(grid), dim3(SBLK), sizeof(int) * 2 * (size_t)max_blocks * (SBLK / 64), s, nn, prp, pcol,
                     perm, x_layout, max_blocks, nullptr, nullptr, lrp, urp, lcol, lsrc, ucol, usrc, isrc, permn);
}
void setup_csr_fill(hipStream_t s, int n, const int *prp, const int *pcol, const int *pdiag, const int *perm, int max_row,
                    const int *lrp, const int *urp, int *lcol, int *lsrc, int *ucol, int *usrc) {
  if (n <= 0) return;
  const int grid = (n + SBLK / 64 - 1) / (SBLK / 64);
  hipLaunchKernelGGL(csr_split_kernel, dim3(grid), dim3(SBLK), sizeof(int) * (size_t)max_row * (SBLK / 64), s, n, prp, pcol, pdiag, perm,
                     max_row, lrp, urp, lcol, lsrc, ucol, usrc);
}

}
```

### navier_stokes_solver_amd/solver.py

```python
from __future__ import annotations

import ctypes as C
import os

import numpy as np

_HERE = os.path.dirname(os.path.abspath(__file__))
_LIB = None

BLK_F, BLK_BT, BLK_B, BLK_MP, BLK_BT_GHOST, BLK_S = range(6)
SPACE_U, SPACE_P = 0, 1
GMRES, FGMRES, BICGSTAB = 0, 1, 2
BLOCK_DIAGONAL, BLOCK_TRIANGULAR, ASIMPLE = 0, 1, 2
STATIONARY, UNSTEADY = 0, 1
TRI_VELOCITY, TRI_PRESSURE = 0, 1
OPT_TRI_ORDERING, OPT_SUBDOMAINS, OPT_FUSE_BLOCK_ROW, OPT_STREAM_KERNELS = 0, 1, 2, 3
OPT_INNER_FUSED_GS, OPT_OUTER_FUSED_GS, OPT_BSR_VELOCITY = 4, 5, 7
OPT_TRI_SYNC_FREE = 9
OPT_VELOCITY_AMG = 10
OPT_CG_SINGLE_REDUCTION = 11
IOPT_TRI_X_LAYOUT, IOPT_FAULT_INJECT, IOPT_TINY_BYTES = 6, 100, 102
OPT_TRI_LINE_GROUPS, IOPT_GROUP_U, IOPT_GROUP_P = 12, 103, 104
OPT_MASS_ORDERING = 13
OPT_BLAS1_PAIRS = 15
OPT_SCHUR_SIGN = 14
OPT_FACTOR_PRECISION = 16
OPT_INNER_MATRIX_PRECISION = 17
OPT_INNER_BASIS_PRECISION = 18
OPT_AMG_PRECISION = 20
OPT_INNER_MATRIX_FREE_F = 19
TIMEOP_MATFREE_F = 56
TIMEOP_INNER_SPMV = 50
IOPT_FUSED_MGS, IOPT_OVERLAP_HALO = 106, 107
IOPT_TIMEOP_BETWEEN = 109
IOPT_INDEX16 = 110
IOPT_GS_ONE_LAUNCH = 111
IOPT_FGMRES_SKIP_UNUSED = 112
IOPT_HOST_ANALYSIS = 108
ORDER_NATURAL, ORDER_MULTICOLOR = 0, 1

EXPORTS = [
    "nsk_get_unique_id", "nsk_local_group_id", "nsk_create", "nsk_destroy", "nsk_last_error", "nsk_set_partition", "nsk_set_halo_plan",
    "nsk_set_support_points",
    "nsk_set_block_csr", "nsk_update_values", "nsk_set_option", "nsk_setup_preconditioner", "nsk_solve",
    "nsk_upload_system", "nsk_solve_resident", "nsk_download_solution", "nsk_spmv", "nsk_jacobian_vmult", "nsk_dot", "nsk_vec_op",
    "nsk_tri_apply", "nsk_amg_info", "nsk_amg_value_bytes", "nsk_tri_get_perm", "nsk_tri_get_value_bytes", "nsk_inner_value_bytes", "nsk_inner_basis_bytes", "nsk_inner_matrix_free", "nsk_matfree_f", "nsk_inner_spmv", "nsk_precond_vmult", "nsk_block_nnz", "nsk_get_block", "nsk_get_stats",
    "nsk_reset_stats", "nsk_get_history", "nsk_cancel", "nsk_abort_group", "nsk_assembly_set_cells", "nsk_assembly_set_simplex", "nsk_assembly_set_dirichlet", "nsk_state_set", "nsk_state_get",
    "nsk_state_save", "nsk_state_save_old", "nsk_state_update", "nsk_assemble", "nsk_scale_values", "nsk_download_rhs", "nsk_time_assemble", "nsk_time_op", "nsk_profile_begin", "nsk_profile_read", "nsk_profile_end",
    "nsk_debug_spmv_form",
    "nsk_forces_set_faces", "nsk_forces_set_edges", "nsk_forces", "nsk_state_get_patches",
    "nsk_record_set_cells", "nsk_state_get_record",
]


class Stats(C.Structure):
    _fields_ = [("setup_ms", C.c_double), ("solve_ms", C.c_double),
                ("outer_iters", C.c_int64), ("inner_u_its", C.c_int64), ("inner_p_its", C.c_int64),
                ("prec_applies", C.c_int64), ("spmv_calls", C.c_int64), ("tri_applies", C.c_int64),
                ("reductions", C.c_int64), ("host_syncs", C.c_int64),
                ("spmv_bytes", C.c_double), ("tri_bytes", C.c_double), ("blas1_bytes", C.c_double),
                ("n_colors_u", C.c_int32), ("n_levels_u", C.c_int32), ("n_colors_p", C.c_int32),
                ("n_levels_p", C.c_int32), ("nnz_s", C.c_int64), ("sync_free_fallbacks", C.c_int64),
                ("cur_outer_iters", C.c_int64), ("cur_residual", C.c_double), ("overlapped_spmvs", C.c_int64),
                ("ring_applies", C.c_int64), ("columns_skipped", C.c_int64)]


class NoConvergence(RuntimeError):

    def __init__(self, status, last_step, last_residual):
        super().__init__(f"solver did not converge (status {status}, step {last_step}, residual {last_residual:g})")
        self.status, self.last_step, self.last_residual = status, last_step, last_residual


def library_path() -> str:
    return os.environ.get("NSK_HIP_LIBRARY") or os.path.join(_HERE, "libnsk_hip.so")


def lib() -> C.CDLL:
    global _LIB
    if _LIB is None:
        path = library_path()
        if not os.path.exists(path):
            raise RuntimeError(f"{path} missing — the HIP extension is required (run __graft_entry__.build())")
        try:
            import torch
        except ImportError:
            pass
        L = C.CDLL(path, mode=C.RTLD_GLOBAL)
        vp, i32p, f64p = C.c_void_p, C.c_void_p, C.c_void_p
        L.nsk_get_unique_id.argtypes = [vp]
        L.nsk_local_group_id.argtypes = [C.c_int, vp]
        L.nsk_create.restype = vp
        L.nsk_create.argtypes = [C.c_int, C.c_int, C.c_int, vp]
        L.nsk_destroy.argtypes = [vp]
        L.nsk_last_error.restype = C.c_char_p
        L.nsk_last_error.argtypes = [vp]
        L.nsk_set_partition.argtypes = [vp, C.c_int, C.c_int64, C.c_int64, C.c_int, i32p]
        L.nsk_set_halo_plan.argtypes = [vp, C.c_int, C.c_int, i32p, i32p, i32p, i32p]
        L.nsk_set_support_points.argtypes = [vp, C.c_int, vp]
        L.nsk_set_block_csr.argtypes = [vp, C.c_int, C.c_int, C.c_int, i32p, i32p, f64p]
        L.nsk_update_values.argtypes = [vp, C.c_int, f64p]
        L.nsk_set_option.argtypes = [vp, C.c_int, C.c_double]
        L.nsk_setup_preconditioner.argtypes = [vp, C.c_int, C.c_int, C.c_double]
        L.nsk_solve.argtypes = [vp, C.c_int, C.c_double, C.c_int, f64p, f64p, f64p, f64p, C.POINTER(C.c_int),
                                C.POINTER(C.c_double)]
        L.nsk_upload_system.argtypes = [vp, f64p, f64p, f64p, f64p]
        L.nsk_solve_resident.argtypes = [vp, C.c_int, C.c_double, C.c_int, C.POINTER(C.c_int), C.POINTER(C.c_double)]
        L.nsk_download_solution.argtypes = [vp, f64p, f64p]
        L.nsk_spmv.argtypes = [vp, C.c_int, f64p, f64p, C.c_int]
        L.nsk_jacobian_vmult.argtypes = [vp, f64p, f64p, f64p, f64p]
        L.nsk_dot.argtypes = [vp, C.c_int, f64p, f64p, C.POINTER(C.c_double), C.POINTER(C.c_double)]
        L.nsk_vec_op.argtypes = [vp, C.c_int, C.c_int, C.c_double, C.c_double, f64p, f64p, f64p, f64p, C.POINTER(C.c_double)]
        L.nsk_assembly_set_cells.argtypes = [vp, C.c_int64, i32p, i32p, vp, f64p, C.c_int32]
        L.nsk_assembly_set_dirichlet.argtypes = [vp, vp, f64p]
        L.nsk_state_set.argtypes = [vp, f64p, f64p]
        L.nsk_state_get.argtypes = [vp, f64p, f64p]
        L.nsk_state_save.argtypes = [vp]
        L.nsk_state_save_old.argtypes = [vp]
# ... 213 lines not shown
        self._ck(self.L.nsk_download_solution(self.h, xu.ctypes.data, xp.ctypes.data))
        return xu, xp

    def spmv(self, blk, x, y=None, add=False, n_rows=None):
        x = _f64(x)
        if n_rows is None:
            n_rows = self.n_u if blk in (BLK_F, BLK_BT) else self.n_p
        out = np.zeros(n_rows) if y is None else _f64(y).copy()
        self._ck(self.L.nsk_spmv(self.h, blk, x.ctypes.data, out.ctypes.data, 1 if add else 0))
        return out

    def jacobian_vmult(self, x_u, x_p):
        xu, xp = _f64(x_u), _f64(x_p)
        yu, yp = np.empty(self.n_u), np.empty(self.n_p)
        self._ck(self.L.nsk_jacobian_vmult(self.h, xu.ctypes.data, xp.ctypes.data, yu.ctypes.data, yp.ctypes.data))
        return yu, yp

    def dot(self, x, y):
        x, y = _f64(x), _f64(y)
        d, nrm = C.c_double(0), C.c_double(0)
        self._ck(self.L.nsk_dot(self.h, len(x), x.ctypes.data, y.ctypes.data, C.byref(d), C.byref(nrm)))
        return d.value, nrm.value

    VEC_OPS = {"copy": 0, "equ": 1, "axpy": 2, "sadd": 3, "axpy2": 4, "scale": 5, "mul": 6, "submul": 7,
               "sub_then_mul": 8, "recip": 9, "axpy_dot": 10, "axpy_norm2": 11}

    def vec_op(self, op, a, c, x, y, z, d):
        x, z, d = _f64(x), _f64(z), _f64(d)
        out = _f64(y).copy()
        sc = C.c_double(0)
        self._ck(self.L.nsk_vec_op(self.h, self.VEC_OPS[op], len(out), a, c, x.ctypes.data, out.ctypes.data, z.ctypes.data,
                                   d.ctypes.data, C.byref(sc)))
        return out, sc.value

    def tri_apply(self, which, b):
        b = _f64(b)
        x = np.empty_like(b)
        self._ck(self.L.nsk_tri_apply(self.h, which, b.ctypes.data, x.ctypes.data))
        return x

    def tri_perm(self, which):
        n = self.n_u if which == TRI_VELOCITY else self.n_p
        p = np.empty(n, np.int32)
        self._ck(self.L.nsk_tri_get_perm(self.h, which, p.ctypes.data))
        return p

    def tri_value_bytes(self, which):
        b = C.c_int32(0)
        self._ck(self.L.nsk_tri_get_value_bytes(self.h, which, C.byref(b)))
        return b.value

    def inner_value_bytes(self, blk):
        b = C.c_int32(0)
        self._ck(self.L.nsk_inner_value_bytes(self.h, blk, C.byref(b)))
        return b.value

    def inner_basis_bytes(self):
        b = C.c_int32(0)
        self._ck(self.L.nsk_inner_basis_bytes(self.h, C.byref(b)))
        return b.value

    def amg_value_bytes(self):
        b = C.c_int32(0)
        self._ck(self.L.nsk_amg_value_bytes(self.h, C.byref(b)))
        return b.value

    def inner_matrix_free(self):
        b = C.c_int32(0)
        self._ck(self.L.nsk_inner_matrix_free(self.h, C.byref(b)))
        return b.value

    def matfree_f(self, x):
        x = _f64(x)
        out = np.zeros(self.n_u)
        self._ck(self.L.nsk_matfree_f(self.h, x.ctypes.data, out.ctypes.data))
        return out

    def index_width(self, blk):
        w = np.zeros(3, np.int32)
        self.L.nsk_debug_index_width.argtypes = [C.c_void_p, C.c_int, C.c_void_p]
        self._ck(self.L.nsk_debug_index_width(self.h, blk, w.ctypes.data))
        return tuple(int(v) for v in w)

    def pool_counts(self):
        w = np.zeros(6, np.int32)
        self.L.nsk_debug_pool_counts.argtypes = [C.c_void_p, C.c_void_p]
        self._ck(self.L.nsk_debug_pool_counts(self.h, w.ctypes.data))
        return tuple((int(w[2 * k]), int(w[2 * k + 1])) for k in range(3))

    def inner_spmv(self, blk, x):
        x = _f64(x)
        out = np.zeros(self.n_u if blk == BLK_F else self.n_p)
        self._ck(self.L.nsk_inner_spmv(self.h, blk, x.ctypes.data, out.ctypes.data))
        return out

    def precond_vmult(self, src_u, src_p, dst_u=None, dst_p=None, calls=1):
        su, sp_ = _f64(src_u), _f64(src_p)
        du = np.zeros(self.n_u) if dst_u is None else _f64(dst_u).copy()
        dp = np.zeros(self.n_p) if dst_p is None else _f64(dst_p).copy()
        rc = self._ck(self.L.nsk_precond_vmult(self.h, su.ctypes.data, sp_.ctypes.data, du.ctypes.data, dp.ctypes.data,
                                               calls), allow=(3,))
        return du, dp, rc

    def get_block(self, blk, n_rows=None):
        nnz = self.L.nsk_block_nnz(self.h, blk)
        if nnz < 0:
            raise RuntimeError("block not present")
        if n_rows is None:
            n_rows = self.n_u if blk in (BLK_F, BLK_BT) else self.n_p
        rp, col, val = np.empty(n_rows + 1, np.int32), np.empty(nnz, np.int32), np.empty(nnz)
        self._ck(self.L.nsk_get_block(self.h, blk, rp.ctypes.data, col.ctypes.data, val.ctypes.data))
        return rp, col, val

    def set_assembly(self, pr, bc_u=None):
        if getattr(pr, "simplex", None) is not None:
            sx = pr.simplex
            arrs = [np.ascontiguousarray(sx[k]) for k in ("cell_u", "cell_p", "grad_lam", "area")]
            lst = [np.ascontiguousarray(sx[k]) for k in ("blk_ptr", "blk_ent", "blk_pos0", "blk_pos1", "node_ptr", "node_ent",
                                                         "vert_ptr", "vert_ent", "outlet_w")]
            self.L.nsk_assembly_set_simplex.argtypes = [C.c_void_p, C.c_int64] + [C.c_void_p] * 4 + [C.c_int64] + \
                [C.c_void_p] * 9 + [C.c_int64]
            self._ck(self.L.nsk_assembly_set_simplex(self.h, len(arrs[0]), *[a.ctypes.data for a in arrs], int(sx["n_blocks"]),
                                                     *[a.ctypes.data for a in lst], int(sx["pos00"])))
            self._keep_simplex = (arrs, lst)
            d = np.ascontiguousarray(pr.dirichlet_u, np.uint8)
            bc = None if bc_u is None else _f64(bc_u)
            self._ck(self.L.nsk_assembly_set_dirichlet(self.h, d.ctypes.data, None if bc is None else bc.ctypes.data))
            return
        cu = np.ascontiguousarray(pr.cell_u_nodes, np.int32)
        cp = np.ascontiguousarray(pr.cell_p_dofs, np.int32)
        cf = np.ascontiguousarray(pr.cell_flags, np.uint8)
        tab = _f64(pr.cell_tables)
        self._ck(self.L.nsk_assembly_set_cells(self.h, cu.shape[0], cu.ctypes.data, cp.ctypes.data, cf.ctypes.data,
                                               tab.ctypes.data, pr.cell_of_dof0))
        d = np.ascontiguousarray(pr.dirichlet_u, np.uint8)
        bc = None if bc_u is None else _f64(bc_u)
        self._ck(self.L.nsk_assembly_set_dirichlet(self.h, d.ctypes.data, None if bc is None else bc.ctypes.data))

    def state_set(self, u, p):
        u, p = _f64(u), _f64(p)
        self._ck(self.L.nsk_state_set(self.h, u.ctypes.data, p.ctypes.data))

    def state_get(self):
        u, p = np.empty(self.n_u), np.empty(self.n_p)
        self._ck(self.L.nsk_state_get(self.h, u.ctypes.data, p.ctypes.data))
        return u, p

    def state_save(self):
        self._ck(self.L.nsk_state_save(self.h))

    def state_save_old(self):
        self._ck(self.L.nsk_state_save_old(self.h))

    def state_update(self, alpha):
        self._ck(self.L.nsk_state_update(self.h, float(alpha)))

    def assemble(self, nu, inv_dt=0.0, p_out=1.0, inhomogeneous_bc=False, stokes=False):
        nrm = C.c_double()
        self._ck(self.L.nsk_assemble(self.h, int(stokes), nu, inv_dt, p_out, int(inhomogeneous_bc), C.byref(nrm)))
        return nrm.value

    def set_forces(self, pr):
        fc = np.ascontiguousarray(pr.face_cell, np.int32)
        fs = np.ascontiguousarray(pr.face_side, np.uint8)
        tab = _f64(pr.face_tables)
        self._ck(self.L.nsk_forces_set_faces(self.h, len(fc), fc.ctypes.data, fs.ctypes.data, tab.ctypes.data))
# ... 100 lines not shown
```

Measured before the change: 10.92 million.

## Compress SpMV column indices into per-run contiguous column intervals

Adds a column-interval encoding for the stream and blocked SpMV plans. Each run of consecutive columns is stored as one 32-bit word (16-bit column offset from a run base plus the entry position), in place of one index per entry. New kernel template variants decode these intervals. The encoding is built only when it is at most 0.75 of the index bytes, so the intent is to cut index traffic in bandwidth-bound SpMV at the cost of decode work and extra setup. Blocked intervals are on by default (col_intervals=1); the 16-bit stream form needs option value 2.

Result: no change. 11.07 million (median of 6 runs) (+1.4%).

```diff
diff --git a/navier_stokes_solver_amd/csrc/nsk_capi.cpp b/navier_stokes_solver_amd/csrc/nsk_capi.cpp
--- a/navier_stokes_solver_amd/csrc/nsk_capi.cpp
+++ b/navier_stokes_solver_amd/csrc/nsk_capi.cpp
@@ -151,6 +151,7 @@
   if (b == NSK_BLK_F) A.build_blocked(2, 2, h->s());
   if (b == NSK_BLK_BT) A.build_blocked(2, 1, h->s());
   if (b == NSK_BLK_B) A.build_blocked(1, 2, h->s());
+  A.build_blk_intervals(h->s(), h->col_intervals >= 1);
   h->ctx.sync();
   if (b == NSK_BLK_F || b == NSK_BLK_BT) { h->jrow_ok = h->jblk_ok = false; h->jrow_nblk = h->jblk_nblk = 0; }
   if (b == NSK_BLK_F) {
@@ -227,6 +228,10 @@
         if (h->blk[b].present && h->blk[b].stream_ok) h->index16_for(h->blk[b], b == NSK_BLK_S ? "S" : "M_p");
       h->ctx.sync();
       h->tS_ok = h->tMp_ok = false;
+      break;
+    case NSK_IOPT_COL_INTERVALS:
+      if (v != 0.0 && v != 1.0 && v != 2.0) throw Error(-61, "NSK_IOPT_COL_INTERVALS: 0, 1 or 2");
+      h->col_intervals = (int)v;
       break;
     case NSK_IOPT_HOST_ANALYSIS:
       h->tF.host_analysis = h->tS.host_analysis = h->tMp.host_analysis = v != 0.0;
diff --git a/navier_stokes_solver_amd/csrc/nsk_core.cpp b/navier_stokes_solver_amd/csrc/nsk_core.cpp
--- a/navier_stokes_solver_amd/csrc/nsk_core.cpp
+++ b/navier_stokes_solver_amd/csrc/nsk_core.cpp
@@ -592,15 +592,19 @@
   const int *cb = off16.p ? colbase.p + c0 : nullptr;
   switch (f) {
     case SpmvForm::blk_f32:
-      nsk::spmv_blk_stream(s, blk_view32(), blk_rowblk.p + c0, c1 - c0, xo, xg, y, mode == 2 ? z : nullptr);
+      nsk::spmv_blk_stream(s, blk_view32(), blk_rowblk.p + c0, c1 - c0, xo, xg, y, mode == 2 ? z : nullptr, blk_iv.view(c0));
       return 0;
-    case SpmvForm::blk: nsk::spmv_blk_stream(s, blk_view(), blk_R, blk_C, blk_rowblk.p + c0, c1 - c0, xo, xg, y); return 0;
+    case SpmvForm::blk:
+      nsk::spmv_blk_stream(s, blk_view(), blk_R, blk_C, blk_rowblk.p + c0, c1 - c0, xo, xg, y, nullptr, nullptr, blk_iv.view(c0));
+      return 0;
     case SpmvForm::stream_f32: {
       const int vec = nsk::spmv_stream(s, view32(), rowblk.p + c0, c1 - c0, even_rows, xo, xg, y, off16.p, cb, mode, z);
       if (vec < 0) throw Error(-1, "fp32 stream SpMV: modes 1 and 2 have no kernel on 16-bit column offsets");
       return vec;
     }
-    default: return nsk::spmv_stream(s, view(), rowblk.p + c0, c1 - c0, even_rows, xo, xg, y, mode, z, off16.p, cb);
+    default:
+      return nsk::spmv_stream(s, view(), rowblk.p + c0, c1 - c0, even_rows, xo, xg, y, mode, z, off16.p, cb,
+                              off16.p ? iv.view(c0) : ColIv());
   }
 }
 
@@ -686,12 +690,62 @@
   off16.release();
   colbase.release();
   idx16_wide = false;
+  iv.release();
+}
+
+void ColIntervals::build(hipStream_t s, int n_runs, const int *rowblk, const int *rowptr, const int *col, int n_own,
+                         int64_t entries, double index_bytes, bool want, bool force) {
+  release();
+  if (!want || n_runs <= 0 || entries <= 0 || !rowblk || !rowptr || !col) return;
+  DBuf<int> flag, cnt;
+  flag.alloc(1);
+  cnt.alloc((size_t)n_runs);
+  base.alloc((size_t)n_runs);
+  NSK_HIP(hipMemsetAsync(flag.p, 0, sizeof(int), s));
+  nsk::setup_run_col_base(s, n_runs, nullptr, rowblk, rowptr, col, base.p, flag.p);
+  nsk::setup_run_interval_counts(s, n_runs, rowblk, rowptr, col, n_own, cnt.p);
+  int w = 0;
+  std::vector<int> hp((size_t)n_runs + 1, 0);
+  NSK_HIP(hipMemcpyAsync(&w, flag.p, sizeof(int), hipMemcpyDeviceToHost, s));
+  NSK_HIP(hipMemcpyAsync(hp.data() + 1, cnt.p, sizeof(int) * (size_t)n_runs, hipMemcpyDeviceToHost, s));
+  NSK_HIP(hipStreamSynchronize(s));
+  if (w) {
+    release();
+    wide = true;
+    return;
+  }
+  int64_t total = 0;
+  for (int b = 0; b < n_runs; ++b) total += hp[(size_t)b + 1];
+  if (total > INT32_MAX) { release(); return; }
+  for (int b = 0; b < n_runs; ++b) hp[(size_t)b + 1] += hp[(size_t)b];
+  count = total;
+  nb = n_runs;
+  pays = bytes() <= kColIvPays * index_bytes;
+  if (!pays && !force) {
+    base.release();
+    return;
+  }
+  ptr.upload(hp, s);
+  word.alloc((size_t)total);
+  nsk::setup_run_intervals(s, n_runs, rowblk, rowptr, col, n_own, base.p, ptr.p, word.p);
+  NSK_HIP(hipStreamSynchronize(s));
+}
+
+void Csr::build_intervals(hipStream_t s, bool want, bool force) {
+  iv.build(s, stream_ok && off16.p ? nblk : 0, rowblk.p, rowptr.p, col.p, n_own_cols, nnz, 2.0 * (double)nnz + 4.0 * nblk, want, force);
+  if (want && idx16_wide) iv.wide = true;
+}
+
+void Csr::build_blk_intervals(hipStream_t s, bool want, bool force) {
+  blk_iv.build(s, blk_ok ? blk_nblk : 0, blk_rowblk.p, blk_rowptr.p, blk_col.p, n_own_cols / std::max(1, blk_C), blk_count,
+               4.0 * (double)blk_count, want, force);
 }
 
 void Csr::build_index16(hipStream_t s, bool want) {
   off16.release();
   colbase.release();
   idx16_wide = false;
+  iv.release();
   if (!want || !stream_ok || nblk <= 0) return;
   if (nnz <= 0) {
     colbase.alloc((size_t)nblk);
@@ -721,6 +775,7 @@
 
 void Csr::build_blocked(int R, int C, hipStream_t s) {
   blk_ok = false;
+  blk_iv.release();
   if (n_rows <= 0 || n_rows % R || n_own_cols % C || n_cols % C) return;
   const int nr = n_rows / R;
   std::vector<int> rp(nr + 1, 0);
diff --git a/navier_stokes_solver_amd/csrc/nsk_core.hpp b/navier_stokes_solver_amd/csrc/nsk_core.hpp
--- a/navier_stokes_solver_amd/csrc/nsk_core.hpp
+++ b/navier_stokes_solver_amd/csrc/nsk_core.hpp
@@ -119,6 +119,21 @@
   if (stream_ok) return SpmvForm::stream_f32;
   return SpmvForm::csr_vector;
 }
+
+constexpr double kColIvPays = 0.75;
+struct ColIntervals {
+  DBuf<unsigned> word;
+  DBuf<int> ptr, base;
+  int64_t count = 0;
+  int nb = 0;
+  bool wide = false, pays = false;
+  bool active() const { return word.p != nullptr; }
+  void release() { word.release(); ptr.release(); base.release(); count = 0; nb = 0; wide = pays = false; }
+  double bytes() const { return 4.0 * (double)count + 8.0 * (double)nb; }
+  ColIv view(int c0) const { return active() ? ColIv{word.p, ptr.p + c0, base.p + c0} : ColIv(); }
+  void build(hipStream_t s, int n_runs, const int *rowblk, const int *rowptr, const int *col, int n_own, int64_t entries,
+             double index_bytes, bool want, bool force);
+};
 
 struct Csr {
   int n_rows = 0, n_cols = 0, n_own_cols = 0;
@@ -137,6 +152,9 @@
   DBuf<int> colbase;
   bool idx16_wide = false;
   void build_index16(hipStream_t s, bool want);
+  ColIntervals iv, blk_iv;
+  void build_intervals(hipStream_t s, bool want, bool force = false);
+  void build_blk_intervals(hipStream_t s, bool want, bool force = false);
   int int_r0 = 0, int_r1 = 0, int_b0 = 0, int_b1 = 0, blk_int_b0 = 0, blk_int_b1 = 0;
   void find_interior();
   bool blk_ok = false;
@@ -173,8 +191,11 @@
                   const double *z = nullptr, int c0 = 0, int c1 = kToPlanEnd) const;
   double format_bytes(SpmvForm f) const {
     const double vb = is_f32(f) ? 4.0 : 8.0;
-    if (is_blk(f)) return (double)blk_count * (4.0 + vb * blk_R * blk_C) + 4.0 * (blk_rows + 1.0) + 8.0 * n_rows + 8.0 * n_cols;
+    if (is_blk(f))
+      return (double)blk_count * vb * blk_R * blk_C + (blk_iv.active() ? blk_iv.bytes() : 4.0 * (double)blk_count) +
+             4.0 * (blk_rows + 1.0) + 8.0 * n_rows + 8.0 * n_cols;
     const bool index16 = off16.p && f != SpmvForm::csr_vector;
+    if (index16 && iv.active() && f == SpmvForm::stream) return (double)spmv_bytes() - 4.0 * (double)nnz + iv.bytes();
     return (double)spmv_bytes() - (8.0 - vb) * (double)nnz - (index16 ? 2.0 * (double)nnz - 4.0 * nblk : 0.0);
   }
   size_t spmv_bytes() const {
diff --git a/navier_stokes_solver_amd/csrc/nsk_debug.cpp b/navier_stokes_solver_amd/csrc/nsk_debug.cpp
--- a/navier_stokes_solver_amd/csrc/nsk_debug.cpp
+++ b/navier_stokes_solver_amd/csrc/nsk_debug.cpp
@@ -335,6 +335,8 @@
   hipStream_t st = h->s();
   for (int k = 0; k < 16; ++k) info[k] = 0;
   info[0] = -1;
+  const bool civ = (form & NSK_DBG_SPMV_COL_INTERVALS) != 0;
+  form &= ~NSK_DBG_SPMV_COL_INTERVALS;
   if (form < NSK_DBG_SPMV_CSRV || form > NSK_DBG_SPMV_BLK22_RES_F32) throw Error(-65, "nsk_debug_spmv: unknown form");
   const bool two = form == NSK_DBG_SPMV_STREAM2 || form == NSK_DBG_SPMV_BLK_FUSED;
   const bool res = form == NSK_DBG_SPMV_BLK22_RES || form == NSK_DBG_SPMV_BLK22_RES_F32;
@@ -350,6 +352,8 @@
   if (form == NSK_DBG_SPMV_BLK21 || epi) R = 2;
   if (form == NSK_DBG_SPMV_BLK12) C = 2;
   const bool blocked = form >= NSK_DBG_SPMV_BLK22 && form != NSK_DBG_SPMV_STREAM2 && form != NSK_DBG_SPMV_STREAM_I16 && form != NSK_DBG_SPMV_STREAM_I16_F32;
+  if (civ && !(form == NSK_DBG_SPMV_STREAM_I16 || (blocked && !two)))
+    throw Error(-61, "nsk_debug_spmv: column intervals exist for the 16-bit stream form and the one-matrix blocked forms");
   if ((misalign & 4) && R == 2) throw Error(-61, "nsk_debug_spmv: the R = 2 forms store pairs, y is 16-byte aligned");
   if (two && Bm->n_rows != Am->n_rows) throw Error(-61, "nsk_debug_spmv: both matrices over the same rows");
 
@@ -380,6 +384,10 @@
     if (!refused && i16) {
       A.build_index16(st, true);
       if (!A.off16.p) refused = 5;
+      else if (civ) {
+        A.build_intervals(st, true, true);
+        if (!A.iv.active()) refused = 6;
+      }
     }
   } else if (form == NSK_DBG_SPMV_STREAM2) {
     if (!A.even_rows) refused = 3;
@@ -393,7 +401,16 @@
     else if (two) {
       if (!fused_blk_plan(A, B, rb)) refused = 4;
       else { ea = &A.h_blk_rowptr; eb = &B.h_blk_rowptr; fused_rb.upload(rb, st); d_rb = fused_rb.p; ib1 = (int)rb.size() - 1; }
-    } else { download(A.blk_rowblk, A.blk_nblk); ea = &A.h_blk_rowptr; ib0 = A.blk_int_b0; ib1 = A.blk_int_b1; }
+    } else {
+      download(A.blk_rowblk, A.blk_nblk);
+      ea = &A.h_blk_rowptr;
+      ib0 = A.blk_int_b0;
+      ib1 = A.blk_int_b1;
+      if (civ) {
+        A.build_blk_intervals(st, true, true);
+        if (!A.blk_iv.active()) refused = 6;
+      }
+    }
   }
   info[15] = refused;
   if (refused) return 1;
@@ -448,7 +465,7 @@
       A.spmv_launch(st, SpmvForm::blk_f32, xa.p, xag.p, yv.p, 0, nullptr, c0, c1);
       break;
     case NSK_DBG_SPMV_BLK22_RES:
-      nsk::spmv_blk22_residual(st, A.blk_view(), d_rb + c0, n_run, xa.p, xag.p, yv.p, zv.p);
+      nsk::spmv_blk22_residual(st, A.blk_view(), d_rb + c0, n_run, xa.p, xag.p, yv.p, zv.p, A.blk_iv.view(c0));
       break;
     case NSK_DBG_SPMV_BLK22_RES_F32:
       A.amg32 = 1;
@@ -456,7 +473,7 @@
       A.spmv_launch(st, SpmvForm::blk_f32, xa.p, xag.p, yv.p, 2, zv.p, c0, c1);
       break;
     case NSK_DBG_SPMV_BLK21_EPI:
-      nsk::spmv_blk_stream(st, A.blk_view(), 2, 1, d_rb + c0, n_run, xa.p, xag.p, yv.p, dv.p, div.p);
+      nsk::spmv_blk_stream(st, A.blk_view(), 2, 1, d_rb + c0, n_run, xa.p, xag.p, yv.p, dv.p, div.p, A.blk_iv.view(c0));
       break;
     case NSK_DBG_SPMV_STREAM2:
       info[1] = nsk::spmv2_stream(st, A.view(), xa.p, xag.p, B.view(), xb.p, xbg.p, d_rb, nblk, yv.p);
@@ -466,11 +483,59 @@
       break;
   }
   NSK_HIP(hipGetLastError());
-  info[0] = form;
+  info[0] = form | (civ ? NSK_DBG_SPMV_COL_INTERVALS : 0);
   info[14] = form == NSK_DBG_SPMV_CSRV ? 0 : n_run;
   int bad = yv.fetch(y, c);
   for (DbgVec<double> *v : {&xa, &xag, &xb, &xbg, &zv, &dv, &div}) bad += v->fetch(nullptr, c);
   info[13] = bad;
+  return 0;
+  NSK_CATCH(h)
+}
+
+int nsk_debug_col_intervals(nsk_handle h, const nsk_dbg_spmv_mat *Am, int blk, int R, int C, int force, int32_t *rowblk_out,
+                            int32_t *ptr_out, int32_t *base_out, int run_cap, uint32_t *word_out, int64_t word_cap,
+                            int64_t *info8) {
+  NSK_TRY_DEV(h)
+  hipStream_t st = h->s();
+  for (int k = 0; k < 8; ++k) info8[k] = 0;
+  if (R < 0 || R > 2 || C < 0 || C > 2 || (R == 0) != (C == 0)) throw Error(-61, "nsk_debug_col_intervals: R, C");
+  Csr tmp;
+  const Csr *A = nullptr;
+  if (Am) {
+    dbg_fill_csr(tmp, *Am, st);
+    if (R) {
+      tmp.build_blocked(R, C, st);
+      tmp.build_blk_intervals(st, true, force != 0);
+    } else {
+      tmp.build_index16(st, true);
+      tmp.build_intervals(st, true, force != 0);
+    }
+    A = &tmp;
+  } else {
+    if (blk < 0 || blk > NSK_BLK_S || !h->blk[blk].present) throw Error(-60, "nsk_debug_col_intervals: block not set");
+    A = &h->blk[blk];
+  }
+  const bool blocked = R != 0;
+  const ColIntervals &T = blocked ? A->blk_iv : A->iv;
+  const bool plan = blocked ? A->blk_ok : A->stream_ok;
+  const int nb = !plan ? 0 : blocked ? A->blk_nblk : A->nblk;
+  info8[0] = T.active();
+  info8[1] = T.wide;
+  info8[2] = T.pays;
+  info8[3] = T.count;
+  info8[4] = nb;
+  info8[5] = blocked ? A->blk_count : A->nnz;
+  info8[6] = plan;
+  info8[7] = blocked ? A->blk_R * 2 + A->blk_C : 0;
+  const size_t nr = (size_t)std::min(nb + 1, std::max(0, run_cap));
+  if (plan && rowblk_out && nr) NSK_HIP(hipMemcpyAsync(rowblk_out, (blocked ? A->blk_rowblk : A->rowblk).p, sizeof(int) * nr, hipMemcpyDeviceToHost, st));
+  if (T.active()) {
+    if (ptr_out && nr) NSK_HIP(hipMemcpyAsync(ptr_out, T.ptr.p, sizeof(int) * nr, hipMemcpyDeviceToHost, st));
+    if (base_out && nr) NSK_HIP(hipMemcpyAsync(base_out, T.base.p, sizeof(int) * std::min(nr, (size_t)nb), hipMemcpyDeviceToHost, st));
+    const size_t nw = (size_t)std::min<int64_t>(T.count, std::max<int64_t>(0, word_cap));
+    if (word_out && nw) NSK_HIP(hipMemcpyAsync(word_out, T.word.p, sizeof(unsigned) * nw, hipMemcpyDeviceToHost, st));
+  }
+  h->ctx.sync();
   return 0;
   NSK_CATCH(h)
 }
diff --git a/navier_stokes_solver_amd/csrc/nsk_handle.hpp b/navier_stokes_solver_amd/csrc/nsk_handle.hpp
--- a/navier_stokes_solver_amd/csrc/nsk_handle.hpp
+++ b/navier_stokes_solver_amd/csrc/nsk_handle.hpp
@@ -291,8 +291,10 @@
     ctx.st.spmv_bytes += (double)A.spmv_bytes() + (mode == 1 ? 8.0 * A.n_rows : 0.0);
   }
   bool index16 = true;
+  int col_intervals = 1;
   void index16_for(Csr &A, const char *name) {
     A.build_index16(s(), index16);
+    A.build_intervals(s(), col_intervals >= 2);
     if (verbose() && index16 && A.stream_ok && !A.off16.p)
       fprintf(stderr, "[nsk] %s: a run of the stream plan spans 65 536 columns or more — int32 column ids stay in use\n", name);
   }
diff --git a/navier_stokes_solver_amd/csrc/nsk_internal.h b/navier_stokes_solver_amd/csrc/nsk_internal.h
--- a/navier_stokes_solver_amd/csrc/nsk_internal.h
+++ b/navier_stokes_solver_amd/csrc/nsk_internal.h
@@ -13,6 +13,7 @@
   NSK_IOPT_INDEX16 = 110,
   NSK_IOPT_GS_ONE_LAUNCH = 111,
   NSK_IOPT_FGMRES_SKIP_UNUSED = 112,
+  NSK_IOPT_COL_INTERVALS = 113,
   NSK_IOPT_FUSED_MGS = 106
 };
 
@@ -43,7 +44,8 @@
   NSK_DBG_SPMV_CSRV = 0, NSK_DBG_SPMV_STREAM = 1, NSK_DBG_SPMV_STREAM_F32 = 2, NSK_DBG_SPMV_BLK22 = 3,
   NSK_DBG_SPMV_BLK21 = 4, NSK_DBG_SPMV_BLK12 = 5, NSK_DBG_SPMV_BLK11 = 6, NSK_DBG_SPMV_BLK22_F32 = 7,
   NSK_DBG_SPMV_BLK21_EPI = 8, NSK_DBG_SPMV_STREAM2 = 9, NSK_DBG_SPMV_BLK_FUSED = 10, NSK_DBG_SPMV_STREAM_I16 = 11,
-  NSK_DBG_SPMV_STREAM_I16_F32 = 12, NSK_DBG_SPMV_BLK22_RES = 13, NSK_DBG_SPMV_BLK22_RES_F32 = 14
+  NSK_DBG_SPMV_STREAM_I16_F32 = 12, NSK_DBG_SPMV_BLK22_RES = 13, NSK_DBG_SPMV_BLK22_RES_F32 = 14,
+  NSK_DBG_SPMV_COL_INTERVALS = 0x100
 };
 struct nsk_dbg_spmv_mat {
   int32_t n_rows, n_cols, n_own_cols, pad_;
@@ -53,6 +55,9 @@
 int nsk_debug_spmv(struct nsk_handle_s *h, int form, int lpr, int mode, int misalign, int c0, int c1,
                    const struct nsk_dbg_spmv_mat *A, const struct nsk_dbg_spmv_mat *B, double *y, const double *z,
                    const double *d, const double *dinv, int32_t *rowblk_out, int rowblk_cap, int32_t *info16);
+int nsk_debug_col_intervals(struct nsk_handle_s *h, const struct nsk_dbg_spmv_mat *A, int blk, int R, int C, int force,
+                            int32_t *rowblk_out, int32_t *ptr_out, int32_t *base_out, int run_cap, uint32_t *word_out,
+                            int64_t word_cap, int64_t *info8);
 struct nsk_dbg_tri_args {
   int32_t n, kind, ordering, n_sub;
   const int32_t *rowptr, *col;
diff --git a/navier_stokes_solver_amd/csrc/nsk_kernels.h b/navier_stokes_solver_amd/csrc/nsk_kernels.h
--- a/navier_stokes_solver_amd/csrc/nsk_kernels.h
+++ b/navier_stokes_solver_amd/csrc/nsk_kernels.h
@@ -36,9 +36,14 @@
 
 constexpr int kStreamNnz = 2048;
 constexpr int kStreamRows = 64;
+struct ColIv {
+  const unsigned *word = nullptr;
+  const int *ptr = nullptr;
+  const int *base = nullptr;
+};
 int spmv_stream(hipStream_t s, const CsrView &A, const int *rowblk, int nblk, int even_rows, const double *x_own,
                 const double *x_ghost, double *y, int mode, const double *z, const unsigned short *off16 = nullptr,
-                const int *colbase = nullptr);
+                const int *colbase = nullptr, ColIv iv = ColIv());
 int spmv_stream(hipStream_t s, const CsrView32 &A, const int *rowblk, int nblk, int even_rows, const double *x_own,
                 const double *x_ghost, double *y, const unsigned short *off16 = nullptr, const int *colbase = nullptr,
                 int mode = 0, const double *z = nullptr);
@@ -57,11 +62,12 @@
 using BlkView32 = BlkViewT<float>;
 constexpr int kBlkMax = 1024;
 void spmv_blk_stream(hipStream_t s, const BlkView &A, int R, int C, const int *rowblk, int nblk, const double *x_own,
-                     const double *x_ghost, double *y, const double *epi_d = nullptr, const double *epi_dinv = nullptr);
+                     const double *x_ghost, double *y, const double *epi_d = nullptr, const double *epi_dinv = nullptr,
+                     ColIv iv = ColIv());
 void spmv_blk_stream(hipStream_t s, const BlkView32 &A, const int *rowblk, int nblk, const double *x_own,
-                     const double *x_ghost, double *y, const double *z = nullptr);
+                     const double *x_ghost, double *y, const double *z = nullptr, ColIv iv = ColIv());
 void spmv_blk22_residual(hipStream_t s, const BlkView &A, const int *rowblk, int nblk, const double *x_own,
-                         const double *x_ghost, double *y, const double *z);
+                         const double *x_ghost, double *y, const double *z, ColIv iv = ColIv());
 void spmv_blk_fused22_21(hipStream_t s, const BlkView &A, const double *xa_own, const double *xa_ghost,
                          const BlkView &B, const double *xb_own, const double *xb_ghost, const int *rowblk, int nblk,
                          double *y);
@@ -247,6 +253,10 @@
                         int *base, int *wide);
 void setup_run_col_offsets(hipStream_t s, int nb, const int4 *desc, const int *rowblk, const int *rowptr, const int *col,
                            const int *base, unsigned short *off);
+void setup_run_interval_counts(hipStream_t s, int nb, const int *rowblk, const int *rowptr, const int *col, int n_own,
+                               int *count);
+void setup_run_intervals(hipStream_t s, int nb, const int *rowblk, const int *rowptr, const int *col, int n_own,
+                         const int *base, const int *ptr, unsigned *word);
 
 void halo_pack(hipStream_t s, int n, const int *idx, const double *x, double *buf);
 constexpr int kLocalSumMax = 16;
diff --git a/navier_stokes_solver_amd/csrc/nsk_kernels.hip b/navier_stokes_solver_amd/csrc/nsk_kernels.hip
--- a/navier_stokes_solver_amd/csrc/nsk_kernels.hip
+++ b/navier_stokes_solver_amd/csrc/nsk_kernels.hip
@@ -91,11 +91,61 @@
   __device__ __forceinline__ IdxPair(unsigned q, int base) : a(base + (int)(q & 0xffffu)), b(base + (int)(q >> 16)) {}
 };
 
-template <class V, int VEC, class I = int>
+__device__ __forceinline__ void expand_col_intervals(const unsigned *__restrict__ word, int i0, int i1, int n,
+                                                     unsigned short *off) {
+  for (int t = i0 + (int)threadIdx.x; t < i1; t += BLK) {
+    const unsigned q = word[t];
+    const int e1 = t + 1 < i1 ? min((int)(word[t + 1] >> 16), n) : n;
+    unsigned c = q & 0xffffu;
+    for (int e = (int)(q >> 16); e < e1; ++e) off[e] = (unsigned short)c++;
+  }
+  __syncthreads();
+}
+
+template <class V, int VEC, class I = int, bool IV = false>
 __device__ __forceinline__ void stream_products(const I *__restrict__ col, const V *__restrict__ val, int k0,
                                                 int k1, int n_own, const double *__restrict__ xo,
-                                                const double *__restrict__ xg, double *prod, int base = 0) {
-  if (VEC == 3) {
+                                                const double *__restrict__ xg, double *prod, int base = 0,
+                                                const unsigned *__restrict__ ivword = nullptr, int i0 = 0, int i1 = 0,
+                                                unsigned short *ivoff = nullptr) {
+  static_assert(!IV || VEC == 2 || VEC == 3, "column intervals: the pair forms only");
+  if constexpr (IV) {
+    constexpr int U = kStreamNnz / (2 * BLK);
+    typedef V vv2 __attribute__((ext_vector_type(2)));
+    typedef vv2 vd2u __attribute__((aligned(VEC == 2 ? 2 * sizeof(V) : sizeof(V))));
+    const int n = k1 - k0;
+    int c0[U], c1[U];
+    double v0[U], v1[U], x0[U], x1[U];
+#pragma unroll
+    for (int u = 0; u < U; ++u) {
+      const int k = k0 + 2 * ((int)threadIdx.x + u * BLK);
+      if (k + 1 < k1) {
+        const vv2 vi = *reinterpret_cast<const vd2u *>(val + k);
+        v0[u] = (double)vi[0]; v1[u] = (double)vi[1];
+      } else {
+        v0[u] = k < k1 ? (double)val[k] : 0.0; v1[u] = 0.0;
+      }
+    }
+    expand_col_intervals(ivword, i0, i1, n, ivoff);
+#pragma unroll
+    for (int u = 0; u < U; ++u) {
+      const int j = 2 * ((int)threadIdx.x + u * BLK);
+      const unsigned q = j < n ? *reinterpret_cast<const unsigned *>(ivoff + j) : 0u;
+      c0[u] = j < n ? base + (int)(q & 0xffffu) : 0;
+      c1[u] = j + 1 < n ? base + (int)(q >> 16) : 0;
+    }
+#pragma unroll
+    for (int u = 0; u < U; ++u) {
+      x0[u] = *(c0[u] < n_own ? xo + c0[u] : xg + (c0[u] - n_own));
+      x1[u] = *(c1[u] < n_own ? xo + c1[u] : xg + (c1[u] - n_own));
+    }
+#pragma unroll
+    for (int u = 0; u < U; ++u) {
+      const int j = 2 * ((int)threadIdx.x + u * BLK);
+      if (j < n) prod[j] = v0[u] * x0[u];
+      if (j + 1 < n) prod[j + 1] = v1[u] * x1[u];
+    }
+  } else if (VEC == 3) {
     constexpr int U = kStreamNnz / (2 * BLK);
     typedef V vv2 __attribute__((ext_vector_type(2)));
     typedef vv2 vd2u __attribute__((aligned(sizeof(V))));
@@ -185,17 +235,20 @@
   return subwave_sum<RG>(s);
 }
 
-template <class V, int VEC, int MODE, class I = int>
+template <class V, int VEC, int MODE, class I = int, bool IV = false>
 __global__ __launch_bounds__(BLK) void spmv_stream_kernel(CsrViewT<V> A, const int *__restrict__ rowblk,
                                                           const double *__restrict__ xo,
                                                           const double *__restrict__ xg, double *__restrict__ y,
                                                           const double *__restrict__ z,
                                                           const unsigned short *__restrict__ off16 = nullptr,
-                                                          const int *__restrict__ colbase = nullptr) {
+                                                          const int *__restrict__ colbase = nullptr, ColIv iv = ColIv()) {
   __shared__ double prod[kStreamNnz];
+  __shared__ unsigned ivoff[IV ? kStreamNnz / 2 : 1];
   const int r0 = rowblk[blockIdx.x], r1 = rowblk[blockIdx.x + 1];
   constexpr bool I16 = std::is_same<I, unsigned short>::value;
+  static_assert(!IV || I16, "column intervals expand to 16-bit offsets");
   const int base = I16 ? colbase[blockIdx.x] : 0;
+  const int i0 = IV ? iv.ptr[blockIdx.x] : 0, i1 = IV ? iv.ptr[blockIdx.x + 1] : 0;
   const int k0 = A.rowptr[r0], k1 = A.rowptr[r1];
   const int r = r0 + (int)threadIdx.x / RG, lane = threadIdx.x % RG;
   const bool have = r < r1;
@@ -207,7 +260,10 @@
     if (MODE == 1) zv = z ? z[r] : y[r];
     if (MODE == 2) zv = z[r];
   }
-  if constexpr (I16) stream_products<V, VEC, unsigned short>(off16, A.val, k0, k1, A.n_own_cols, xo, xg, prod, base);
+  if constexpr (IV)
+    stream_products<V, VEC, unsigned short, true>(nullptr, A.val, k0, k1, A.n_own_cols, xo, xg, prod, base, iv.word, i0, i1,
+                                                  reinterpret_cast<unsigned short *>(ivoff));
+  else if constexpr (I16) stream_products<V, VEC, unsigned short>(off16, A.val, k0, k1, A.n_own_cols, xo, xg, prod, base);
   else stream_products<V, VEC>(A.col, A.val, k0, k1, A.n_own_cols, xo, xg, prod);
   __syncthreads();
   const double sum = row_sum_lds(prod, jb, je, lane);
@@ -245,9 +301,11 @@
   if (have && lane == 0) y[r] = sum;
 }
 
-template <class V, int R, int C>
+template <class V, int R, int C, bool IV = false>
 __device__ __forceinline__ void blk_products(const BlkViewT<V> &A, int k0, int k1, const double *__restrict__ xo,
-                                             const double *__restrict__ xg, double *p0, double *p1) {
+                                             const double *__restrict__ xg, double *p0, double *p1, int base = 0,
+                                             const unsigned *__restrict__ ivword = nullptr, int i0 = 0, int i1 = 0,
+                                             unsigned short *ivoff = nullptr) {
   constexpr int U = kBlkMax / BLK;
   if (k0 >= k1) return;
   int m[U];
@@ -257,7 +315,7 @@
   for (int u = 0; u < U; ++u) {
     const int k = k0 + (int)threadIdx.x + u * BLK;
     const bool ok = k < k1;
-    m[u] = ok ? __builtin_nontemporal_load(A.col + k) : 0;
+    if constexpr (!IV) m[u] = ok ? __builtin_nontemporal_load(A.col + k) : 0;
     const V *v = A.val + (size_t)(R * C) * (ok ? k : k0);
     if constexpr (std::is_same<V, float>::value) {
       static_assert(R == 2 && C == 2, "fp32 values: 2 x 2 blocks only");
@@ -267,6 +325,14 @@
       if (R * C == 4) { a0[u] = *reinterpret_cast<const double2 *>(v); a1[u] = *reinterpret_cast<const double2 *>(v + 2); }
       else if (R * C == 2) { a0[u] = *reinterpret_cast<const double2 *>(v); a1[u] = make_double2(0.0, 0.0); }
       else { a0[u] = make_double2(v[0], 0.0); a1[u] = make_double2(0.0, 0.0); }
+    }
+  }
+  if constexpr (IV) {
+    expand_col_intervals(ivword, i0, i1, k1 - k0, ivoff);
+#pragma unroll
+    for (int u = 0; u < U; ++u) {
+      const int j = (int)threadIdx.x + u * BLK;
+      m[u] = j < k1 - k0 ? base + (int)ivoff[j] : 0;
     }
   }
 #pragma unroll
@@ -296,20 +362,22 @@
   }
 }
 
-template <class V, int R, int C, int EPI>
-__global__ __launch_bounds__(BLK) void spmv_blk_kernel(BlkViewT<V> A, const int *__restrict__ rowblk,
+template <class V, int R, int C, int EPI, bool IV = false>
+__global__ __launch_bounds__(BLK) __attribute__((amdgpu_waves_per_eu(IV ? 8 : 1))) void spmv_blk_kernel(BlkViewT<V> A, const int *__restrict__ rowblk,
                                                        const double *__restrict__ xo, const double *__restrict__ xg,
                                                        double *__restrict__ y, const double *__restrict__ d,
-                                                       const double *__restrict__ dinv) {
+                                                       const double *__restrict__ dinv, ColIv iv = ColIv()) {
   __shared__ double p0[kBlkMax];
   __shared__ double p1[R == 2 ? kBlkMax : 1];
+  __shared__ unsigned short ivoff[IV ? kBlkMax : 1];
   const int r0 = rowblk[blockIdx.x], r1 = rowblk[blockIdx.x + 1];
+  const int base = IV ? iv.base[blockIdx.x] : 0, i0 = IV ? iv.ptr[blockIdx.x] : 0, i1 = IV ? iv.ptr[blockIdx.x + 1] : 0;
   const int k0 = A.rowptr[r0], k1 = A.rowptr[r1];
   const int r = r0 + (int)threadIdx.x / RG, lane = threadIdx.x % RG;
   const bool have = r < r1;
   int jb = 0, je = 0;
   if (have) { jb = A.rowptr[r] - k0; je = A.rowptr[r + 1] - k0; }
-  blk_products<V, R, C>(A, k0, k1, xo, xg, p0, p1);
+  blk_products<V, R, C, IV>(A, k0, k1, xo, xg, p0, p1, base, iv.word, i0, i1, ivoff);
   __syncthreads();
   double s0 = 0.0, s1 = 0.0;
   for (int j = jb + lane; j < je; j += RG) { s0 += p0[j]; if (R == 2) s1 += p1[j]; }
@@ -1515,11 +1583,13 @@
 }
 
 int spmv_stream(hipStream_t s, const CsrView &A, const int *rowblk, int nblk, int even_rows, const double *xo,
-                const double *xg, double *y, int mode, const double *z, const unsigned short *off16, const int *colbase) {
+                const double *xg, double *y, int mode, const double *z, const unsigned short *off16, const int *colbase,
+                ColIv iv) {
   if (nblk <= 0) return 0;
 #define NSK_SS(V, M)                                                                                                                   \
   do {                                                                                                                                 \
-    if (off16) hipLaunchKernelGGL((spmv_stream_kernel<double, V, M, unsigned short>), dim3(nblk), dim3(BLK), 0, s, A, rowblk, xo, xg, y, z, off16, colbase); \
+    if (iv.word) hipLaunchKernelGGL((spmv_stream_kernel<double, V, M, unsigned short, true>), dim3(nblk), dim3(BLK), 0, s, A, rowblk, xo, xg, y, z, nullptr, iv.base, iv); \
+    else if (off16) hipLaunchKernelGGL((spmv_stream_kernel<double, V, M, unsigned short>), dim3(nblk), dim3(BLK), 0, s, A, rowblk, xo, xg, y, z, off16, colbase); \
     else hipLaunchKernelGGL((spmv_stream_kernel<double, V, M, int>), dim3(nblk), dim3(BLK), 0, s, A, rowblk, xo, xg, y, z, off16, colbase); \
   } while (0)
   if (even_rows) {
@@ -1579,13 +1649,18 @@
 }
 
 void spmv_blk_stream(hipStream_t s, const BlkView &A, int R, int C, const int *rowblk, int nblk, const double *xo,
-                     const double *xg, double *y, const double *epi_d, const double *epi_dinv) {
+                     const double *xg, double *y, const double *epi_d, const double *epi_dinv, ColIv iv) {
   if (nblk <= 0) return;
   if (epi_d) {
-    hipLaunchKernelGGL((spmv_blk_kernel<double, 2, 1, 1>), dim3(nblk), dim3(BLK), 0, s, A, rowblk, xo, xg, y, epi_d, epi_dinv);
+    if (iv.word) hipLaunchKernelGGL((spmv_blk_kernel<double, 2, 1, 1, true>), dim3(nblk), dim3(BLK), 0, s, A, rowblk, xo, xg, y, epi_d, epi_dinv, iv);
+    else hipLaunchKernelGGL((spmv_blk_kernel<double, 2, 1, 1>), dim3(nblk), dim3(BLK), 0, s, A, rowblk, xo, xg, y, epi_d, epi_dinv, iv);
     return;
   }
-#define NSK_BK(RR, CC) hipLaunchKernelGGL((spmv_blk_kernel<double, RR, CC, 0>), dim3(nblk), dim3(BLK), 0, s, A, rowblk, xo, xg, y, nullptr, nullptr)
+#define NSK_BK(RR, CC)                                                                                                                 \
+  do {                                                                                                                                 \
+    if (iv.word) hipLaunchKernelGGL((spmv_blk_kernel<double, RR, CC, 0, true>), dim3(nblk), dim3(BLK), 0, s, A, rowblk, xo, xg, y, nullptr, nullptr, iv); \
+    else hipLaunchKernelGGL((spmv_blk_kernel<double, RR, CC, 0>), dim3(nblk), dim3(BLK), 0, s, A, rowblk, xo, xg, y, nullptr, nullptr, iv); \
+  } while (0)
   if (R == 2 && C == 2) NSK_BK(2, 2);
   else if (R == 2 && C == 1) NSK_BK(2, 1);
   else if (R == 1 && C == 2) NSK_BK(1, 2);
@@ -1594,16 +1669,19 @@
 }
 
 void spmv_blk_stream(hipStream_t s, const BlkView32 &A, const int *rowblk, int nblk, const double *xo, const double *xg,
-                     double *y, const double *z) {
+                     double *y, const double *z, ColIv iv) {
   if (nblk <= 0) return;
-  if (z) hipLaunchKernelGGL((spmv_blk_kernel<float, 2, 2, 2>), dim3(nblk), dim3(BLK), 0, s, A, rowblk, xo, xg, y, z, nullptr);
-  else hipLaunchKernelGGL((spmv_blk_kernel<float, 2, 2, 0>), dim3(nblk), dim3(BLK), 0, s, A, rowblk, xo, xg, y, nullptr, nullptr);
+#define NSK_BK(E, IVM) hipLaunchKernelGGL((spmv_blk_kernel<float, 2, 2, E, IVM>), dim3(nblk), dim3(BLK), 0, s, A, rowblk, xo, xg, y, z, nullptr, iv)
+  if (z) { if (iv.word) NSK_BK(2, true); else NSK_BK(2, false); }
+  else { if (iv.word) NSK_BK(0, true); else NSK_BK(0, false); }
+#undef NSK_BK
 }
 
 void spmv_blk22_residual(hipStream_t s, const BlkView &A, const int *rowblk, int nblk, const double *xo, const double *xg,
-                         double *y, const double *z) {
-  if (nblk > 0)
-    hipLaunchKernelGGL((spmv_blk_kernel<double, 2, 2, 2>), dim3(nblk), dim3(BLK), 0, s, A, rowblk, xo, xg, y, z, nullptr);
+                         double *y, const double *z, ColIv iv) {
+  if (nblk <= 0) return;
+  if (iv.word) hipLaunchKernelGGL((spmv_blk_kernel<double, 2, 2, 2, true>), dim3(nblk), dim3(BLK), 0, s, A, rowblk, xo, xg, y, z, nullptr, iv);
+  else hipLaunchKernelGGL((spmv_blk_kernel<double, 2, 2, 2>), dim3(nblk), dim3(BLK), 0, s, A, rowblk, xo, xg, y, z, nullptr, iv);
 }
 
 void spmv_blk_fused22_21(hipStream_t s, const BlkView &A, const double *xao, const double *xag, const BlkView &B,
diff --git a/navier_stokes_solver_amd/csrc/nsk_setup_kernels.hip b/navier_stokes_solver_amd/csrc/nsk_setup_kernels.hip
--- a/navier_stokes_solver_amd/csrc/nsk_setup_kernels.hip
+++ b/navier_stokes_solver_amd/csrc/nsk_setup_kernels.hip
@@ -143,6 +143,52 @@
     if (k0 < k1 && (long long)mx - (long long)mn > 65535) *wide = 1;
   }
 }
+template <int FILL>
+__global__ __launch_bounds__(SBLK) void run_intervals_kernel(int nb, const int *__restrict__ rowblk, const int *__restrict__ rowptr,
+                                                             const int *__restrict__ col, int n_own, const int *__restrict__ base,
+                                                             int *__restrict__ count, const int *__restrict__ ptr,
+                                                             unsigned *__restrict__ word) {
+  __shared__ int part[SBLK];
+  const int b = (int)blockIdx.x;
+  if (b >= nb) return;
+  const int k0 = rowptr[rowblk[b]], k1 = rowptr[rowblk[b + 1]], n = k1 - k0;
+  const int per = (n + SBLK - 1) / SBLK;
+  const int a = min(n, (int)threadIdx.x * per), e = min(n, a + per);
+  auto opens = [&](int j) {
+    if (j == 0) return true;
+    const int c = col[k0 + j];
+    return c != col[k0 + j - 1] + 1 || c == n_own;
+  };
+  int mine = 0;
+  for (int j = a; j < e; ++j) mine += opens(j) ? 1 : 0;
+  part[threadIdx.x] = mine;
+  __syncthreads();
+  if (!FILL) {
+    if (threadIdx.x == 0) {
+      int total = 0;
+      for (int t = 0; t < SBLK; ++t) total += part[t];
+      count[b] = total;
+    }
+    return;
+  }
+  int before = 0;
+  for (int t = 0; t < (int)threadIdx.x; ++t) before += part[t];
+  unsigned *w = word + ptr[b] + before;
+  const int bs = base[b];
+  for (int j = a; j < e; ++j)
+    if (opens(j)) *w++ = (unsigned)(col[k0 + j] - bs) | (unsigned)j << 16;
+}
+}
+
+void setup_run_interval_counts(hipStream_t s, int nb, const int *rowblk, const int *rowptr, const int *col, int n_own,
+                               int *count) {
+  if (nb <= 0) return;
+  hipLaunchKernelGGL((run_intervals_kernel<0>), dim3(nb), dim3(SBLK), 0, s, nb, rowblk, rowptr, col, n_own, nullptr, count, nullptr, nullptr);
+}
+void setup_run_intervals(hipStream_t s, int nb, const int *rowblk, const int *rowptr, const int *col, int n_own,
+                         const int *base, const int *ptr, unsigned *word) {
+  if (nb <= 0) return;
+  hipLaunchKernelGGL((run_intervals_kernel<1>), dim3(nb), dim3(SBLK), 0, s, nb, rowblk, rowptr, col, n_own, base, nullptr, ptr, word);
 }
 
 void setup_run_col_base(hipStream_t s, int nb, const int4 *desc, const int *rowblk, const int *rowptr, const int *col,
diff --git a/navier_stokes_solver_amd/solver.py b/navier_stokes_solver_amd/solver.py
--- a/navier_stokes_solver_amd/solver.py
+++ b/navier_stokes_solver_amd/solver.py
@@ -34,6 +34,7 @@
 IOPT_FUSED_MGS, IOPT_OVERLAP_HALO = 106, 107
 IOPT_TIMEOP_BETWEEN = 109
 IOPT_INDEX16 = 110
+IOPT_COL_INTERVALS = 113
 IOPT_GS_ONE_LAUNCH = 111
 IOPT_FGMRES_SKIP_UNUSED = 112
 IOPT_HOST_ANALYSIS = 108
@@ -413,6 +414,14 @@
         self._ck(self.L.nsk_debug_index_width(self.h, blk, w.ctypes.data))
         return tuple(int(v) for v in w)
 
+    def col_intervals(self, blk, blocked):
+        info = np.zeros(8, np.int64)
+        self.L.nsk_debug_col_intervals.argtypes = [C.c_void_p, C.c_void_p] + [C.c_int] * 4 + [C.c_void_p] * 3 + [C.c_int, C.c_void_p, C.c_int64, C.c_void_p]
+        rc = 1 if blocked else 0
+        self._ck(self.L.nsk_debug_col_intervals(self.h, None, blk, rc, rc, 0, None, None, None, 0, None, 0, info.ctypes.data))
+        return dict(active=bool(info[0]), wide=bool(info[1]), pays=bool(info[2]), intervals=int(info[3]), runs=int(info[4]),
+                    entries=int(info[5]), plan=bool(info[6]))
+
     def pool_counts(self):
         w = np.zeros(6, np.int32)
         self.L.nsk_debug_pool_counts.argtypes = [C.c_void_p, C.c_void_p]
```
